# viiika/Diffusion-Conductor

Measured on AMD Instinct MI355X. Metric: motion frames/sec (DDIM-50, 60s clip, bs=32 per GPU), higher is better.
Workload: dtype f16; 1 GPU; configs[1]: DDIM-50 sampling loop, bs=32 clips/GPU x 1800 frames (60 s), linear attention, precision=fp16, conditioning + x_T resident in HBM (loop-only); clips_per_gpu=32, frames_per_clip=1800, ddim_steps=50, parallelism=clip-dp1, precise_tail_steps=1

## Files before the change

### diffusion-conductor_amd/csrc/dc_api.hip

```cpp
#include <hip/hip_runtime.h>

#include <algorithm>
#include <cmath>
#include <cstdarg>
#include <cstdio>
#include <cstdlib>
#include <cstring>
#include <map>
#include <string>
#include <tuple>
#include <vector>

#include "../../include/dc_ddim.h"
#include "dc_common.h"
#include "dc_form.h"
#include "dc_launch.h"
#include "dc_music.h"
#include "dc_pack.h"

namespace {

thread_local std::string g_err;

int fail(int code, const char* fmt, ...) {
// ... 33 lines not shown
    DcModel* d_model = nullptr;
    DcModel h_model{};
    int NT = 0;

    hipStream_t stream = nullptr;
    hipEvent_t ev_in = nullptr, ev_out = nullptr;

    int B = 0, T = 0, M = 0, G = 0;
    int Tx = 0;
    size_t cap_G = 0, cap_B = 0, cap_MP = 0, cap_steps = 0, cap_snap = 0, cap_kv = 0;
    size_t cap_rec_floats = 0;
    std::vector<int> len_dev;
    const int* len_dev_ptr = nullptr;
    int* d_length = nullptr;
    float* d_pp = nullptr;
    void *d_s_hi = nullptr, *d_s_lo = nullptr;
    void* d_E = nullptr;
    float* d_h = nullptr;
    float* d_recs = nullptr;
    void *d_a_sa = nullptr, *d_a_ca = nullptr;
    void* d_a_ca16 = nullptr;
    unsigned long long* d_gran = nullptr;
    unsigned l16_seq = 0;
    bool l16_own = false;
    void *d_kv_sa[2] = {nullptr, nullptr}, *d_kv_ca = nullptr;
    int KT = 0;
    float* d_x = nullptr;
    float* d_snaps = nullptr;
    float* d_recs_ca = nullptr;
    void *d_nh_hi = nullptr, *d_nh_lo = nullptr;
    unsigned long long* d_stamps = nullptr;
    float* d_film_rate = nullptr;
    int film_rate_parity = 0;
    int num_cu = 0;
    int *d_iter = nullptr, *d_t_clip = nullptr, *d_snap_cur = nullptr, *d_t_of_iter = nullptr, *d_snap_of_iter = nullptr;
    float *d_coef_cur = nullptr, *d_coef_of_iter = nullptr;
    bool cond_set = false;
    int64_t ws_bytes = 0;
    std::map<void*, size_t> alloc_bytes;
    int tables_S = 0;
    std::vector<int> tab_t, tab_snap;
    std::vector<float> tab_coef_iter;

    std::vector<std::pair<GraphKey, hipGraphExec_t>> graphs;
    int upd_flags = 0;
    const float** d_zslot = nullptr;
    float* d_zstep = nullptr;
    size_t cap_zstep = 0;
    unsigned long long noise_seed = 0, noise_first = 0;
    bool noise_seed_set = false;
    int* d_status = nullptr;
    float* d_x0_prev = nullptr;
    size_t cap_x0_prev = 0;
    const float *known_val = nullptr, *known_mask = nullptr, *known_noise = nullptr;
    struct KnownFor {
        int user_B = 0, Tx = 0;
        bool guided = false;
        int takes = 1;
        bool operator==(const KnownFor& o) const { return user_B == o.user_B && Tx == o.Tx && guided == o.guided && takes == o.takes; }
    } known_set_for;
    KnownFor known_for() const { return {user_B(), Tx, guided, takes}; }
    const float** d_kslot = nullptr;
    int smooth_window = 0, smooth_order = 0, smooth_table_window = 0;
    float* d_smooth_coef = nullptr;
    bool guided = false;
    float guide_w = 1.f;
    float* d_wslot = nullptr;
    float* d_raw = nullptr;
    size_t cap_raw = 0;
    float *d_xf2_proj = nullptr, *d_xf2_out = nullptr;
    size_t cap_xf2_proj = 0, cap_xf2_out = 0;
    int user_B() const { return guided ? B / 2 : B; }
    int takes = 1;
    float* d_pp_share = nullptr;
    size_t cap_pp_share = 0;
    const float* pp_last = nullptr;
    int last_film_groups = 0;

    DcModel h_model_split{};
    DcModel* d_model_split = nullptr;
    dc_music* music = nullptr;
    int me_format = -1;
    int clip_aligned = -1;
    bool precise_forward = false;
    int tail_split = -1;
    bool host_only = false;

    Prof prof;
    bool diag_film_done = false;
};

namespace {

template <class P>
int dev_alloc(dc_sampler* s, P*& p, size_t bytes) {
    if (p) {
        auto it = s->alloc_bytes.find((void*)p);
        if (it != s->alloc_bytes.end()) {
            s->ws_bytes -= (int64_t)it->second;
            s->alloc_bytes.erase(it);
        }
        void* old = (void*)p;
        p = nullptr;
        HIP_TRY(hipFree(old));
    }
    void* q = nullptr;
    HIP_TRY(hipMalloc(&q, bytes));
    p = (P*)q;
    s->alloc_bytes[q] = bytes;
    s->ws_bytes += (int64_t)bytes;
    return DC_OK;
}

void drop_graph(dc_sampler* s) {
    for (auto& g : s->graphs) hipGraphExecDestroy(g.second);
    s->graphs.clear();
}

template <class P>
int grow(dc_sampler* s, P*& p, size_t& cap, size_t need, size_t elem_bytes, bool in_graphs) {
    if (need <= cap) return DC_OK;
    if (in_graphs) drop_graph(s);
    cap = 0;
    if (int rc = dev_alloc(s, p, need * elem_bytes)) return rc;
    cap = need;
    return DC_OK;
}

const std::vector<float>* find(dc_sampler* s, const std::string& n) {
    auto it = s->params.find(n);
    return it == s->params.end() ? nullptr : &it->second;
}

struct ParamReq {
    std::string name;
    size_t numel;
};

std::vector<ParamReq> required_params(const dc_config& c) {
    std::vector<ParamReq> r;
    const size_t D = c.latent_dim, E = 4 * D, L = 512, F = c.ff_size, P = c.input_feats;
    r.push_back({"sequence_embedding", (size_t)c.num_frames * D});
    r.push_back({"linear.weight", L * 64});
    r.push_back({"linear.bias", L});
    r.push_back({"joint_embed.weight", D * P});
    r.push_back({"joint_embed.bias", D});
    r.push_back({"time_embed.0.weight", E * D});
    r.push_back({"time_embed.0.bias", E});
    r.push_back({"time_embed.2.weight", E * E});
    r.push_back({"time_embed.2.bias", E});
    auto styl = [&](const std::string& p) {
        r.push_back({p + ".emb_layers.1.weight", 2 * D * E});
        r.push_back({p + ".emb_layers.1.bias", 2 * D});
        r.push_back({p + ".norm.weight", D});
        r.push_back({p + ".norm.bias", D});
        r.push_back({p + ".out_layers.2.weight", D * D});
        r.push_back({p + ".out_layers.2.bias", D});
    };
    for (int i = 0; i < c.num_layers; ++i) {
        const std::string p = "temporal_decoder_blocks." + std::to_string(i);
        r.push_back({p + ".sa_block.norm.weight", D});
        r.push_back({p + ".sa_block.norm.bias", D});
        for (const char* n : {"query", "key", "value"}) {
            r.push_back({p + ".sa_block." + n + ".weight", D * D});
            r.push_back({p + ".sa_block." + n + ".bias", D});
        }
// ... 292 lines not shown
        add_image(I.top(&DcModel::img_out), P("out.weight"), P_, DC_D, true, ob.data(), ob.size());
        std::vector<float> ob16(32, 0.f);
        for (int k = 0; k < P_; ++k) ob16[k] = P("out.bias")[k];
        add_image16(I.top(&DcModel::out16), P("out.weight"), P_, DC_D, nullptr, 0, 0, true, ob16);
    }
    void conditioning_front(const LinearStats& lin) {
        const float* w = P("linear.weight");
        std::vector<float> wt((size_t)64 * 512);
        for (int k = 0; k < 512; ++k)
            for (int x = 0; x < 64; ++x) wt[(size_t)x * 512 + k] = w[(size_t)k * 64 + x];
        add_vec(I.top(&DcModel::lin_wt), wt);
        add_vec(I.top(&DcModel::lin_b), P("linear.bias"), 512);
        add_vec(I.top(&DcModel::lin_gram), lin.gram);
        add_natural(I.top(&DcModel::lin_pack), w, 512, 64, false);
    }
    void time_embedding() {
        add_vec(I.top(&DcModel::temb), std::vector<float>((size_t)c.max_timesteps * 512, 0.f));
        std::vector<float> fr(64);
        for (int k = 0; k < 64; ++k) fr[k] = (float)std::exp((double)((float)(-std::log(10000.0)) * (float)k / 64.f));
        std::vector<float> w0t((size_t)128 * 512), w2t((size_t)512 * 512);
        const float* w0 = P("time_embed.0.weight");
        const float* w2 = P("time_embed.2.weight");
        for (int o = 0; o < 512; ++o) {
            for (int x = 0; x < 128; ++x) w0t[(size_t)x * 512 + o] = w0[(size_t)o * 128 + x];
            for (int x = 0; x < 512; ++x) w2t[(size_t)x * 512 + o] = w2[(size_t)o * 512 + x];
        }
        I.freqs = I.arena.add(fr);
        I.w0t = I.arena.add(w0t);
        I.b0 = I.arena.add(P("time_embed.0.bias"), 512 * 4);
        I.w2t = I.arena.add(w2t);
        I.b2 = I.arena.add(P("time_embed.2.bias"), 512 * 4);
    }
};

void pack_model(const dc_config& c, const Formats& fmt, const DcParams& params, ModelImage& I) {
    const int L = c.num_layers;
    I.NT = 3 * L * DC_FILM_TILES_PER_BLOCK;
    I.model.num_layers = L;
    I.model.input_feats = c.input_feats;
    I.model.num_frames = c.num_frames;
    I.model.max_timesteps = c.max_timesteps;
    I.split = I.model;
    ModelPacker k{c, fmt, params, I};
    const LinearStats lin = centre_linear(k.P("linear.weight"), k.P("linear.bias"));
    for (int i = 0; i < L; ++i) k.decoder_layer(i, lin);
    k.film_stack();
    k.pose_projections();
    k.add_vec(I.top(&DcModel::seq_emb), k.P("sequence_embedding"), (size_t)c.num_frames * DC_D);
    k.conditioning_front(lin);
    k.time_embedding();
}

int upload_model(dc_sampler* s, ModelImage& I) {
    const std::vector<uint8_t>& host = I.arena.host;
    s->NT = I.NT;
    s->arena_bytes = host.size();
    if (s->host_only) {
        free(s->d_arena);
        s->d_arena = (uint8_t*)malloc(host.size());
        memcpy(s->d_arena, host.data(), host.size());
    } else {
        if (s->d_arena) hipFree(s->d_arena);
        HIP_TRY(hipMalloc((void**)&s->d_arena, host.size()));
        HIP_TRY(hipMemcpy(s->d_arena, host.data(), host.size(), hipMemcpyHostToDevice));
    }
    I.arena.resolve(s->d_arena);
    s->h_model = I.model;
    s->h_model_split = I.split;
    if (s->host_only) return DC_OK;
    if (!s->d_model) HIP_TRY(hipMalloc((void**)&s->d_model, sizeof(DcModel)));
    HIP_TRY(hipMemcpy(s->d_model, &s->h_model, sizeof(DcModel), hipMemcpyHostToDevice));
    if (!s->d_model_split) HIP_TRY(hipMalloc((void**)&s->d_model_split, sizeof(DcModel)));
    HIP_TRY(hipMemcpy(s->d_model_split, &s->h_model_split, sizeof(DcModel), hipMemcpyHostToDevice));
    const auto op = [&](size_t off) { return (const float*)(s->d_arena + off); };
    HIP_TRY(dc_launch_temb_table(s->stream, op(I.freqs), op(I.w0t), op(I.b0), op(I.w2t), op(I.b2), (float*)s->h_model.temb, s->cfg.max_timesteps));
    HIP_TRY(hipStreamSynchronize(s->stream));
    return DC_OK;
}

Settings settings_of(const dc_sampler* s) {
    Settings r;
    r.precision = s->cfg.precision, r.fmt = *s, r.no_eff = s->cfg.no_eff != 0, r.clip_aligned = s->clip_aligned, r.l16_own = s->l16_own;
    r.num_layers = s->cfg.num_layers, r.split_model = s->d_model_split != nullptr, r.film_w16 = s->h_model.film_w16 != nullptr;
    r.film_w16_tail = s->h_model.film_w16_tail != nullptr, r.l16_max_units = dc_layer16_max_units();
    return r;
}
int clip_stride(const dc_sampler* s, int B, int Tx) { return clip_stride(settings_of(s), Switches::read(), B, Tx, s->num_cu); }
int ensure_workspace(dc_sampler* s, int B, int Tx) {
    const int T = clip_stride(s, B, Tx);
    const int M = B * T, G = cdiv(M, 32), L = s->cfg.num_layers, P = s->cfg.input_feats;
    if ((size_t)G > s->cap_G) {
        drop_graph(s);
        const size_t g = (size_t)G;
        s->cap_G = 0;
        int rc;
        if ((rc = dev_alloc(s, s->d_pp, g * 32 * 64 * 8 * 4))) return rc;
        if ((rc = dev_alloc(s, s->d_s_hi, g * 32 * 64 * 16))) return rc;
        if ((rc = dev_alloc(s, s->d_s_lo, g * 32 * 64 * 16))) return rc;
        if ((rc = dev_alloc(s, s->d_E, g * s->NT * 64 * 32))) return rc;
        if ((rc = dev_alloc(s, s->d_h, g * 4 * 64 * 64))) return rc;
        HIP_TRY(hipMemset(s->d_h, 0, g * 4 * 64 * 64));
        s->cap_rec_floats = rec_capacity(g);
        if ((rc = dev_alloc(s, s->d_recs, s->cap_rec_floats * 4))) return rc;
        if ((rc = dev_alloc(s, s->d_nh_hi, g * 32 * 64 * 16))) return rc;
        if ((rc = dev_alloc(s, s->d_nh_lo, g * 32 * 64 * 16))) return rc;
        if (!s->cfg.no_eff && (rc = dev_alloc(s, s->d_recs_ca, (size_t)L * g * 2 * DC_REC_FLOATS * 4))) return rc;
        s->cap_G = g;
    }
    if (s->cfg.no_eff) {
        const int KT = (T + 31) / 32 + 1;
        const size_t need = (size_t)B * KT;
        if (need > s->cap_kv) {
            drop_graph(s);
            s->cap_kv = 0;
            int rc;
            for (int i = 0; i < 2; ++i)
                if ((rc = dev_alloc(s, s->d_kv_sa[i], need * 16384))) return rc;
            if ((rc = dev_alloc(s, s->d_kv_ca, (size_t)L * need * 16384))) return rc;
            s->cap_kv = need;
        }
        s->KT = KT;
    }
    if ((size_t)B > s->cap_B) {
        drop_graph(s);
        s->cap_B = 0;
        int rc;
        if ((rc = dev_alloc(s, s->d_length, (size_t)B * 4))) return rc;
        if ((rc = dev_alloc(s, s->d_t_clip, (size_t)B * 4))) return rc;
        if ((rc = dev_alloc(s, s->d_a_sa, (size_t)B * 16 * 1024))) return rc;
        if ((rc = dev_alloc(s, s->d_a_ca, (size_t)L * B * 16 * 1024))) return rc;
        if ((rc = dev_alloc(s, s->d_a_ca16, (size_t)L * B * 8 * 1024))) return rc;
        if ((rc = dev_alloc(s, s->d_gran, (size_t)B * 1024 * 8))) return rc;
        HIP_TRY(hipMemset(s->d_gran, 0, (size_t)B * 1024 * 8));
        s->cap_B = (size_t)B;
    }
    if ((size_t)M * P > s->cap_MP) {
        drop_graph(s);
        s->cap_MP = 0;
        int rc;
        if ((rc = dev_alloc(s, s->d_x, (size_t)M * P * 4))) return rc;
        s->cap_MP = (size_t)M * P;
    }
    if (!s->d_iter) {
        int rc;
        if ((rc = dev_alloc(s, s->d_stamps, (8 * 32 + 8 + 1024 + 1024 + 256 + 8 + 512) * 8))) return rc;
        if ((rc = dev_alloc(s, s->d_film_rate, 2 * 1024 * sizeof(float)))) return rc;
        HIP_TRY(hipMemset(s->d_film_rate, 0, 2 * 1024 * sizeof(float)));
        if ((rc = dev_alloc(s, s->d_status, 16))) return rc;
        HIP_TRY(hipMemset(s->d_status, 0, 16));
        if ((rc = dev_alloc(s, s->d_zslot, 32))) return rc;
        HIP_TRY(hipMemset(s->d_zslot, 0, 32));
        if ((rc = dev_alloc(s, s->d_kslot, 32))) return rc;
        HIP_TRY(hipMemset(s->d_kslot, 0, 32));
        if ((rc = dev_alloc(s, s->d_iter, 16))) return rc;
        if ((rc = dev_alloc(s, s->d_snap_cur, 16))) return rc;
        if ((rc = dev_alloc(s, s->d_coef_cur, DC_COEF * 4))) return rc;
    }
    if ((s->B != B || s->T != T) && s->d_gran)
        HIP_TRY(hipMemsetAsync(s->d_gran, 0, s->cap_B * 1024 * 8, s->stream));
    s->B = B;
    s->T = T;
    s->Tx = Tx;
    s->M = M;
    s->G = G;
    return DC_OK;
}

// ... 29 lines not shown
    } while (0)

struct Step : StepOpts {
    const float* x_src = nullptr;
    float* x_dst = nullptr;
};
struct StepDone {
    bool embedded_next = false;
    bool folded = false;
};

DcFilmArgs film_args(const dc_sampler* s, const float* pp, const int* t_clip) {
    DcFilmArgs f{};
    f.W = s->h_model.film_w, f.bias_ft = s->h_model.film_b, f.s_hi = s->d_s_hi, f.s_lo = s->d_s_lo, f.E = s->d_E, f.G = s->G, f.NT = s->NT;
    f.nround = s->NT / 16, f.pp = pp, f.temb = s->h_model.temb, f.t_clip = t_clip, f.T = s->T, f.B = s->B;
    f.W16 = s->h_model.film_w16, f.bias16 = s->h_model.film_b16, f.status = s->d_status;
    return f;
}

int enqueue_step(dc_sampler* s, hipStream_t st, const Step& c, const Switches& w, StepDone* done = nullptr) {
    static const bool want_stamps = getenv("DC_STAMPS") != nullptr;
    const int B = s->B, T = s->T, M = s->M, G = s->G, Tx = s->Tx;
    const StepForm f = step_form(Geometry{B, T, Tx, G, s->num_cu, s->cap_rec_floats}, settings_of(s), w, c, want_stamps);
    const bool folded = f.folded;
    const int fs = f.fs, ff = f.ff, graph_step = c.graph_step;
    const bool ss = f.ss, sf = s->split_film;
    const unsigned l16_tag = folded ? 16u * (unsigned)graph_step : (0x40000000u | (16u * (s->l16_seq++ & 0x3ffffffu)));
    if (!f.error.empty()) return fail(DC_ERR_INVALID, "%s", f.error.c_str());
    if (done) done->embedded_next = f.embed_next, done->folded = folded;
    const DcModel* dmod = (c.split && !s->split_small) ? s->d_model_split : s->d_model;
    const int* iter_base = folded ? s->d_iter : nullptr;
    const int* t_src = folded ? s->d_t_of_iter + graph_step : s->d_t_clip;
    const float* coef_src = folded ? s->d_coef_of_iter + DC_COEF * (size_t)graph_step : s->d_coef_cur;
    const int* snap_src = folded ? s->d_snap_of_iter + graph_step : s->d_snap_cur;
    if (c.loop_mode && !folded)
        LAUNCH(K_BEGIN, dc_launch_begin_step(st, s->d_iter, s->d_t_of_iter, s->d_coef_of_iter, s->d_snap_of_iter,
                                             s->d_t_clip, s->d_coef_cur, s->d_snap_cur, B));
    if (c.loop_mode && (s->upd_flags & DC_UPD_ZSTEP))
        LAUNCH(K_NOISE, dc_launch_step_noise(st, s->d_zstep, (size_t)s->user_B() * Tx * s->cfg.input_feats, 0, reinterpret_cast<const unsigned long long*>(s->d_zslot) + 1,
                                             iter_base, folded ? graph_step : 0,
                                             folded ? nullptr : s->d_snap_cur, 0));
    if (!f.fuse_silu)
        LAUNCH(K_SILU, dc_launch_silu_emb(st, ff, sf, s->d_pp, s->h_model.temb, s->d_t_clip, s->d_s_hi, s->d_s_lo, G, T, B));
    DcEmbedArgs ea{};
    if (f.fuse_embed) ea = DcEmbedArgs{dmod, c.x_src, s->d_h, s->d_recs, s->d_length, M, Tx, f.nwg, f.upc, ss ? 1 : 0, 0};
    if (f.fuse_extra) ea = DcEmbedArgs{s->d_model, c.x_src, s->d_h, s->d_recs, s->d_length, M, Tx, f.nwg, f.upc, 0, 1};
    DcFilmArgs fa = film_args(s, f.fuse_silu ? s->d_pp : nullptr, t_src);
    if (f.g1_tiles) fa.bias_ft = s->h_model.film_b_g1, fa.bias16 = s->h_model.film_b16_g1;
    if (f.film_tail) fa.W16 = s->h_model.film_w16_tail;
    s->last_film_groups = f.film_groups;
    fa.G = f.film_groups;
    if (f.guided && f.film_period < f.film_wrap) {
        if (!s->d_pp_share || (size_t)f.film_groups > s->cap_pp_share) return fail(DC_ERR_INVALID, "internal: no operand image for the shared takes of a guided step");
        fa.pp = s->d_pp_share;
    }
    s->pp_last = fa.pp;
    fa.clk = want_stamps ? s->d_stamps + 252 : nullptr;
    if (f.adapt) fa.rate_in = s->d_film_rate + 1024 * s->film_rate_parity, fa.rate_out = s->d_film_rate + 1024 * (s->film_rate_parity ^ 1);
    fa.iter_base = iter_base;
    fa.embed = (f.fuse_embed || f.fuse_extra) ? &ea : nullptr;
    const bool diag_skip_film = getenv("DC_DIAG_SKIP_FILM") && !f.fuse_embed && !f.fuse_extra && s->diag_film_done;
    s->diag_film_done = true;
    if (!diag_skip_film) LAUNCH(K_FILM, dc_launch_film_gemm(st, ff, sf, fa));
    s->film_rate_parity ^= 1;
    const int nl_run = f.nl_run;
    DcLayerArgs la{};
    la.dm = dmod, la.hbuf = s->d_h, la.E = s->d_E, la.NT = s->NT, la.recs = s->d_recs, la.length = s->d_length, la.xin = c.x_src, la.xout = c.x_dst;
    la.out_mode = (c.loop_mode && !f.guided) ? 1 : 0, la.coef_cur = coef_src, la.snap_cur = snap_src, la.snaps = s->d_snaps, la.iter_base = iter_base;
    la.M = M, la.T = T, la.G = G, la.B = B, la.Tx = Tx, la.e_groups = f.film_groups, la.e_period = f.film_period, la.e_wrap = f.film_wrap, la.e_magic = film_magic(f.film_period, f.film_wrap);
    if (f.guided) la.xout = s->d_raw;
    la.upd = DcUpdate{s->d_zslot, s->d_status, (c.loop_mode ? s->upd_flags : 0) | f.upd_flags, folded ? graph_step : -1, nullptr, s->d_kslot, s->d_x0_prev};
    DcLayerArgs la_stamps = la;
    la_stamps.upd.stamps = s->d_stamps;
    if (s->cfg.no_eff) {
        LAUNCH(K_EMBED, dc_launch_embed_front_full(st, fs, ss, dmod, c.x_src, s->d_h, s->d_kv_sa[0], M, T, B, s->KT));
        for (int l = 0; l < nl_run; ++l)
            LAUNCH(K_LAYER, dc_launch_layer_full(st, fs, ss, (want_stamps && l == 3) ? la_stamps : la, l, s->d_kv_sa[l & 1], s->d_kv_sa[(l + 1) & 1],
                                                 s->d_kv_ca, s->KT, (l == nl_run - 1) ? f.stop_stage : 0));
        if (f.guided)
            LAUNCH(K_GUIDE, dc_launch_guided_update(st, s->d_raw, c.x_dst, (size_t)s->user_B() * Tx * s->cfg.input_feats, coef_src, snap_src,
                                                    s->d_snaps, iter_base, s->d_wslot, la.upd));
        return DC_OK;
    }
    const DcLayerForm lf{fs, ss, f.wgr, f.narrow, f.g1_tiles, f.upc, f.rec_stride};
    if (f.fuse_embed || f.fuse_extra || c.embedded) {
    } else if (c.dbg.first >= 0)
        LAUNCH(K_EMBED, dc_launch_front_from_h(st, fs, ss, dmod, s->d_h, s->d_recs, s->d_length, M, T, G, B, c.dbg.first));
    else
        LAUNCH(K_EMBED, dc_launch_embed_front(st, lf, dmod, c.x_src, s->d_h, s->d_recs, s->d_length, M, T, G, B,
                                              want_stamps ? s->d_stamps + 256 : nullptr, Tx));
    for (int l = c.dbg.first >= 0 ? c.dbg.first : 0; l < nl_run; ++l) {
        if (f.layer16) {
            static const bool stamps16 = getenv("DC_L16_STAMPS") != nullptr;
            LAUNCH(K_LAYER, dc_launch_layer16(st, fs, (stamps16 && l == 3) ? la_stamps : la, l, s->d_a_ca16, f.upc16, f.rec_stride,
                                              l == 0 ? f.upc_narrow : f.upc16, l == 0 ? (size_t)2 * DC_REC_FLOATS : (size_t)DC_REC_FLOATS,
                                              f.l16_shared ? s->d_gran : nullptr, l16_tag, f.g1_tiles));
            continue;
        }
        if (!f.wgr) LAUNCH(K_COMBINE, dc_launch_attn_combine(st, fs, s->d_recs, s->d_a_sa, T, G, B, 1, 32));
        LAUNCH(K_LAYER, dc_launch_layer(st, lf, la, l, s->d_a_sa, s->d_a_ca, (l == nl_run - 1) ? f.stop_stage : 0,
                                        ((l == 3 || l == 4) && want_stamps) ? s->d_stamps : nullptr));
    }
    if (f.guided)
        LAUNCH(K_GUIDE, dc_launch_guided_update(st, s->d_raw, c.x_dst, (size_t)s->user_B() * Tx * s->cfg.input_feats, coef_src, snap_src,
                                                s->d_snaps, iter_base, s->d_wslot, la.upd));
    return DC_OK;
}

int sync_in(dc_sampler* s, hipStream_t user) {
    HIP_TRY(hipEventRecord(s->ev_in, user));
    HIP_TRY(hipStreamWaitEvent(s->stream, s->ev_in, 0));
    return DC_OK;
}
int sync_out(dc_sampler* s, hipStream_t user) {
    HIP_TRY(hipEventRecord(s->ev_out, s->stream));
    HIP_TRY(hipStreamWaitEvent(user, s->ev_out, 0));
    return DC_OK;
}

struct LoopCall {
    const float* d_noise = nullptr;
    float* d_out = nullptr;
    int n = 0;
    bool listed = false;
    const int32_t* h_timesteps = nullptr;
    const float* h_rows = nullptr;
    int flags = 0;
    const float* d_step_noise = nullptr;
    const int32_t* h_snap_iters = nullptr;
    int n_snap = 0;
    float* d_snaps = nullptr;
    bool profile = false;
    float* h_ms = nullptr;
    int32_t* h_count = nullptr;
    int n_kernels = 0;
    void* stream = nullptr;
};

int loop_validate(dc_sampler* s, const LoopCall& c, int& flags) {
    const int S = c.n;
    const float* h_coef = c.h_rows;
    const bool profile = c.profile;
    if (!s || !s->finalized) return fail(DC_ERR_INVALID, "sampler not finalized");
    if (!s->cond_set) return fail(DC_ERR_INVALID, "dc_sampler_set_conditioning must be called first");
    if (S < 1 || S > s->cfg.max_timesteps) return fail(DC_ERR_INVALID, "num_steps %d outside [1, max_timesteps=%d]", S, s->cfg.max_timesteps);
    if (!c.d_noise || !c.d_out || !h_coef) return fail(DC_ERR_INVALID, "null pointer argument");
    if ((flags & DC_UPD_EPS) && s->cfg.no_eff && !(flags & DC_UPD_NOISY) && !getenv("DC_ALLOW_EPSILON_NO_EFF_ETA0"))
        return fail(DC_ERR_UNSUPPORTED, "EPSILON model with full attention (no_eff) at eta = 0 is outside the 1e-3 parity bound (up to 1.3e-3); "
                                        "use linear attention, or eta > 0");
    if (s->known_mask && !(s->known_set_for == s->known_for())) s->known_val = s->known_mask = s->known_noise = nullptr;
    const bool known = s->known_mask != nullptr;
    if (known && S > 1 && !(h_coef[5] > 0.f))
        return fail(DC_ERR_INVALID, "known values are set: the loop needs the [S][8] table of dc_ddim_coefficients_known (slot 5 = sqrt(1 - abar_prev))");
    if (known && profile) return fail(DC_ERR_UNSUPPORTED, "dc_sampler_profile_loop does not run with known values set");
    if (known) flags |= DC_UPD_KNOWN;
    if (s->smooth_window > 0 && s->Tx < s->smooth_window)
        return fail(DC_ERR_INVALID, "smoothing window %d exceeds the %d frames of a clip", s->smooth_window, s->Tx);
    return DC_OK;
}

int loop_prepare(dc_sampler* s, const LoopCall& c, int& flags, size_t MP) {
    const int S = c.n, n_snap = c.n_snap;
    const int32_t *h_t = c.h_timesteps, *h_snap_iters = c.h_snap_iters;
    const float* h_coef = c.h_rows;
    int rc;
    if ((rc = ensure_steps(s, S))) return rc;
    if ((rc = grow(s, s->d_snaps, s->cap_snap, (size_t)n_snap * MP, 4, true))) return rc;
// ... 512 lines not shown
    int rc;
    if ((rc = grow(s, s->d_xf2_proj, s->cap_xf2_proj, irows * 64, 4, false))) return rc;
    if ((rc = grow(s, s->d_xf2_out, s->cap_xf2_out, irows * 64, 4, false))) return rc;
    hipStream_t user = (hipStream_t)stream;
    for (int j = 0; j < takes; ++j) {
        HIP_TRY(hipMemcpyAsync(s->d_xf2_proj + (size_t)j * rows * 64, d_xf_proj, rows * 64 * 4, hipMemcpyDeviceToDevice, user));
        HIP_TRY(hipMemcpyAsync(s->d_xf2_out + (size_t)j * rows * 64, d_xf_out, rows * 64 * 4, hipMemcpyDeviceToDevice, user));
    }
    if (guided) {
        DcNull64 np{}, no{};
        memcpy(np.v, h_null_proj, sizeof np.v);
        memcpy(no.v, h_null_out, sizeof no.v);
        HIP_TRY(dc_launch_fill_rows64(user, s->d_xf2_proj + crows * 64, crows, np));
        HIP_TRY(dc_launch_fill_rows64(user, s->d_xf2_out + crows * 64, crows, no));
    }
    std::vector<int32_t> len2;
    if (h_length)
        for (long long j = 0; j < Bi / B; ++j) len2.insert(len2.end(), h_length, h_length + B);
    if ((rc = set_conditioning(s, s->d_xf2_proj, s->d_xf2_out, h_length ? len2.data() : nullptr, (int)Bi, T, stream))) return rc;
    s->cond_set = false;
    if (guided) {
        if ((rc = grow(s, s->d_raw, s->cap_raw, irows * s->cfg.input_feats, 4, true))) return rc;
        if (!s->d_wslot && (rc = dev_alloc(s, s->d_wslot, 16))) return rc;
        s->guide_w = 1.f;
        const FilmShare sh = film_share(s->B, s->T, s->G, true, takes, !s->split_film, Switches{});
        if (sh.period < sh.wrap) {
            const size_t gbytes = (size_t)32 * 64 * 8 * 4;
            if ((rc = grow(s, s->d_pp_share, s->cap_pp_share, (size_t)sh.groups, gbytes, true))) return rc;
            char* dst = reinterpret_cast<char*>(s->d_pp_share);
            const char* src = reinterpret_cast<const char*>(s->d_pp);
            HIP_TRY(hipMemcpyAsync(dst, src, (size_t)sh.period * gbytes, hipMemcpyDeviceToDevice, user));
            HIP_TRY(hipMemcpyAsync(dst + (size_t)sh.period * gbytes, src + (size_t)sh.wrap * gbytes, gbytes, hipMemcpyDeviceToDevice, user));
        }
    }
    s->guided = guided;
    s->takes = takes;
    s->cond_set = true;
    return DC_OK;
}

int dc_sampler_set_conditioning_guided(dc_sampler* s, const float* d_xf_proj, const float* d_xf_out, const int32_t* h_length, int32_t B,
                                       int32_t T, const float* h_null_proj, const float* h_null_out, void* stream) {
    if (!s || !s->finalized) return fail(DC_ERR_INVALID, "sampler not finalized");
    if (!h_null_proj || !h_null_out) return fail(DC_ERR_INVALID, "guided conditioning: the null pair (h_null_proj[64], h_null_out[64]) is NULL");
    return set_conditioning_images(s, d_xf_proj, d_xf_out, h_length, B, T, 1, h_null_proj, h_null_out, stream);
}

int dc_sampler_set_conditioning_takes(dc_sampler* s, const float* d_xf_proj, const float* d_xf_out, const int32_t* h_length, int32_t B,
                                      int32_t T, int32_t takes, const float* h_null_proj, const float* h_null_out, void* stream) {
    if (!s || !s->finalized) return fail(DC_ERR_INVALID, "sampler not finalized");
    if (takes < 1) return fail(DC_ERR_INVALID, "takes=%d: a conditioning holds at least one take per music", takes);
    if ((h_null_proj != nullptr) != (h_null_out != nullptr))
        return fail(DC_ERR_INVALID, "takes: the null pair is both vectors (guided) or neither (unguided); one of h_null_proj, h_null_out is NULL");
    if (takes == 1 && !h_null_proj) return dc_sampler_set_conditioning(s, d_xf_proj, d_xf_out, h_length, B, T, stream);
    return set_conditioning_images(s, d_xf_proj, d_xf_out, h_length, B, T, takes, h_null_proj, h_null_out, stream);
}

int dc_sampler_set_guidance_scale(dc_sampler* s, float w) {
    if (!s) return fail(DC_ERR_INVALID, "null sampler");
    if (!std::isfinite(w)) return fail(DC_ERR_INVALID, "guidance scale must be finite");
    if (!s->guided) return fail(DC_ERR_INVALID, "dc_sampler_set_conditioning_guided must be called first: the scale belongs to a guided conditioning");
    s->guide_w = w;
    return DC_OK;
}

int dc_sampler_set_precise_tail(dc_sampler* s, int32_t steps) {
    if (!s) return fail(DC_ERR_INVALID, "null sampler");
    if (steps < -1) return fail(DC_ERR_INVALID, "precise tail: steps >= 0, or -1 for the precision's default");
    s->tail_split = steps;
    return DC_OK;
}

int32_t dc_precise_tail_default(int32_t precision) {
    return precise_tail_default(precision);
}

int dc_sampler_set_clip_aligned(dc_sampler* s, int32_t mode) {
    if (!s) return fail(DC_ERR_INVALID, "null sampler");
    if (mode < -1 || mode > 1) return fail(DC_ERR_INVALID, "clip-aligned units: 1 (always), 0 (flat units), -1 (the library's rule)");
    s->clip_aligned = mode;
    return DC_OK;
}

int dc_sampler_set_precise_forward(dc_sampler* s, int32_t on) {
    if (!s) return fail(DC_ERR_INVALID, "null sampler");
    s->precise_forward = on != 0;
    return DC_OK;
}

int dc_sampler_set_combine_exchange(dc_sampler* s, int32_t on) {
    if (!s) return fail(DC_ERR_INVALID, "null sampler");
    s->l16_own = on == 0;
    return DC_OK;
}

int dc_sampler_set_encoder_format(dc_sampler* s, int32_t format) {
    if (!s) return fail(DC_ERR_INVALID, "null sampler");
    if (format != DC_ME_SPLIT && format != DC_ME_FP16) return fail(DC_ERR_INVALID, "encoder format %d (DC_ME_SPLIT = 0, DC_ME_FP16 = 1)", format);
    s->me_format = format;
    if (s->music) dc_music_set_format(s->music, format);
    return DC_OK;
}

int dc_sampler_encode_music(dc_sampler* s, const float* d_mel, int32_t B, int32_t Tm, int32_t n_mels, float* d_xf_proj,
                            float* d_xf_out, void* stream) {
    if (!s || !s->finalized) return fail(DC_ERR_INVALID, "sampler not finalized");
    if (!s->music) return fail(DC_ERR_PARAM, "music encoder parameters (music_encoder.*, proj.*) were not supplied");
    if (!d_mel || !d_xf_proj || !d_xf_out || B < 1) return fail(DC_ERR_INVALID, "bad encode_music arguments");
    if (n_mels != 128) return fail(DC_ERR_UNSUPPORTED, "mel spectrograms must have 128 bins (conv4 takes 32 channels x 16 bins), got %d", n_mels);
    if (Tm < 4) return fail(DC_ERR_INVALID, "need at least 4 mel frames (reflection padding of the (Tm - 1) / 3 + 1 rows behind the stride-3 pool), got %d", Tm);
    HIP_TRY(hipSetDevice(s->cfg.device));
    hipStream_t user = (hipStream_t)stream, st = s->stream;
    int rc;
    if ((rc = sync_in(s, user))) return rc;
    std::string err;
    const hipError_t e = dc_music_encode(s->music, d_mel, B, Tm, d_xf_proj, d_xf_out, st, &err);
    if (e != hipSuccess) return fail(DC_ERR_HIP, "encode_music: %s %s", hipGetErrorString(e), err.c_str());
    return sync_out(s, user);
}

int dc_savgol_coefficients(int32_t window, int32_t order, float* h_coef) {
    if (window < 3 || !(window & 1) || window > 99 || order < 0 || order >= window || order > 10 || !h_coef)
        return fail(DC_ERR_INVALID, "savgol: need an odd window in [3,99] and 0 <= order < window (order <= 10)");
    const int w = window, n = order + 1, hw = w / 2;
    std::vector<double> A((size_t)w * n), G((size_t)n * n, 0.0), Ginv((size_t)n * n, 0.0);
    for (int i = 0; i < w; ++i) {
        const double u = (double)(i - hw) / hw;
        double pw = 1.0;
        for (int j = 0; j < n; ++j) {
            A[(size_t)i * n + j] = pw;
            pw *= u;
        }
    }
    for (int a = 0; a < n; ++a)
        for (int b = 0; b < n; ++b) {
            double acc = 0.0;
            for (int i = 0; i < w; ++i) acc += A[(size_t)i * n + a] * A[(size_t)i * n + b];
            G[(size_t)a * n + b] = acc;
        }
    std::vector<double> M((size_t)n * 2 * n, 0.0);
    for (int a = 0; a < n; ++a) {
        for (int b = 0; b < n; ++b) M[(size_t)a * 2 * n + b] = G[(size_t)a * n + b];
        M[(size_t)a * 2 * n + n + a] = 1.0;
    }
    for (int c = 0; c < n; ++c) {
        int piv = c;
        for (int r = c + 1; r < n; ++r)
            if (std::fabs(M[(size_t)r * 2 * n + c]) > std::fabs(M[(size_t)piv * 2 * n + c])) piv = r;
        if (std::fabs(M[(size_t)piv * 2 * n + c]) < 1e-300) return fail(DC_ERR_INVALID, "savgol: singular normal equations");
        if (piv != c)
            for (int k = 0; k < 2 * n; ++k) std::swap(M[(size_t)piv * 2 * n + k], M[(size_t)c * 2 * n + k]);
        const double d = M[(size_t)c * 2 * n + c];
        for (int k = 0; k < 2 * n; ++k) M[(size_t)c * 2 * n + k] /= d;
        for (int r = 0; r < n; ++r)
            if (r != c) {
                const double f = M[(size_t)r * 2 * n + c];
                if (f != 0.0)
                    for (int k = 0; k < 2 * n; ++k) M[(size_t)r * 2 * n + k] -= f * M[(size_t)c * 2 * n + k];
            }
    }
    for (int a = 0; a < n; ++a)
        for (int b = 0; b < n; ++b) Ginv[(size_t)a * n + b] = M[(size_t)a * 2 * n + n + b];
    for (int i = 0; i < w; ++i)
        for (int k = 0; k < w; ++k) {
            double acc = 0.0;
            for (int a = 0; a < n; ++a) {
// ... 243 lines not shown
```

### diffusion-conductor_amd/csrc/dc_form.h

```cpp
#pragma once
#include <algorithm>
#include <cstdio>
#include <cstdlib>
#include <optional>
#include <string>
#include <tuple>
#include <vector>

#include "dc_common.h"

constexpr int DCF_BF16 = 0, DCF_MIXED = 1, DCF_BF16X3 = 2, DCF_FP16 = 3;

struct Formats {
    int small_fmt = 0, film_fmt = 0;
    bool split_small = false, split_film = false;
    void set_precision(int precision) {
        split_small = precision == DCF_MIXED || precision == DCF_BF16X3;
        split_film = precision == DCF_BF16X3;
        small_fmt = precision == DCF_FP16 ? 1 : 0;
        film_fmt = (precision == DCF_FP16 || precision == DCF_MIXED) ? 1 : 0;
    }
};

#define DC_FORM_SWITCHES(X)                                                                                                            \
    X(no_wgrec, "DC_NO_WGREC") X(no_narrow, "DC_NO_NARROW") X(no_align, "DC_NO_ALIGN") X(align, "DC_ALIGN")                          \
    X(no_fuse_embed, "DC_NO_FUSE_EMBED") X(film_static, "DC_FILM_STATIC") X(begin_step, "DC_BEGIN_STEP") X(no_pad, "DC_NO_PAD")      \
    X(no_layer16, "DC_NO_LAYER16") X(l16_own_combine, "DC_L16_OWN_COMBINE") X(l16_test_drop_slice, "DC_L16_TEST_DROP_SLICE")         \
    X(tail_film_bf16, "DC_TAIL_FILM_BF16") X(flat_units, "DC_FLAT_UNITS") X(no_embed_next, "DC_NO_EMBED_NEXT")                  \
    X(guide_full_film, "DC_GUIDE_FULL_FILM") X(takes_full_film, "DC_TAKES_FULL_FILM")
struct Switches {
#define X(field, name) bool field = false;
    DC_FORM_SWITCHES(X)
#undef X
    static Switches read() {
        Switches w;
#define X(field, name) w.field = getenv(name) != nullptr;
        DC_FORM_SWITCHES(X)
#undef X
        return w;
    }
    unsigned long long bits() const {
        unsigned long long k = 0;
        int i = 0;
#define X(field, name) k |= (field ? 1ull : 0ull) << i++;
        DC_FORM_SWITCHES(X)
#undef X
        return k;
    }
};

inline size_t rec_capacity(size_t g) { return std::max(g * 2, 4 * ((g + 3) / 4) + 8) * DC_REC_FLOATS; }

struct Geometry {
    int B = 0, T = 0, Tx = 0, G = 0;
    int num_cu = 0;
    size_t cap_rec_floats = 0;
};

inline unsigned long long guided_key_bits(bool guided, bool shared_film) {
    return (guided ? 1ull << 27 : 0ull) | ((guided && shared_film) ? 1ull << 28 : 0ull);
}

struct Settings {
    int precision = DCF_FP16;
    Formats fmt;
    bool no_eff = false;
    int clip_aligned = -1;
    bool l16_own = false;
    int num_layers = 0;
    bool split_model = false;
    bool film_w16 = false, film_w16_tail = false;
    int l16_max_units = 0;
};

struct Hooks {
    int layers = -1, stage = 0;
    int first = -1;
    bool production() const { return layers < 0 && stage == 0 && first < 0; }
};

struct StepOpts {
    bool loop_mode = false;
    int graph_step = -1;
    bool split = false;
    bool g1_loop = false;
    bool next_plain = false;
    bool embedded = false;
    bool profile = false;
    bool known = false;
    int takes = 1;
    bool guided = false;
    Hooks dbg;
};

struct StepForm {
    std::string error;
    bool ss = false;
    bool film_tail = false;
    int fs = 0, ff = 0;
    bool fuse_silu = false;
    bool folded = false;
    bool adapt = false;
    bool wgr = false, narrow = false, aligned = false, layer16 = false, l16_shared = false;
    int upc = 0, upc16 = 0, upc_narrow = 0, nwg = 0;
    size_t rec_stride = 0;
    bool mixed_form = false, embed_next = false, fuse_embed = false, fuse_extra = false, g1_tiles = false;
    int upd_flags = 0;
    int nl_run = 0, stop_stage = 0;
    bool guided = false;
    bool shared_film = false;
    int film_groups = 0;
    int film_period = 0, film_wrap = 0;
};

struct FilmShare {
    int period = 0, wrap = 0, groups = 0;
};
inline FilmShare film_share(int B, int T, int G, bool guided, int takes, bool film_from_pp, const Switches& w) {
    const FilmShare full{G, G, G};
    const int Bc = guided ? B / 2 : B;
    if ((guided && B % 2) || takes < 1 || Bc % takes || !film_from_pp || (guided && w.guide_full_film)) return full;
    const long long mc = (long long)(Bc / takes) * T;
    if (mc % 32 != 0) return full;
    const long long gc = mc / 32, wrap = gc * takes;
    if ((guided ? 2 * wrap : wrap) != G) return full;
    const int period = (int)((takes > 1 && !w.takes_full_film && gc >= 2 && wrap * gc < (1ll << 32)) ? gc : wrap), groups = period + (guided ? 1 : 0);
    return groups < G ? FilmShare{period, (int)wrap, groups} : full;
}
inline unsigned film_magic(int period, int wrap) { return period < wrap ? (unsigned)((1ull << 32) / (unsigned)period) + 1u : 0u; }
inline int takes_key_period(const FilmShare& f) { return f.period < f.wrap ? f.period : 0; }

inline bool can_split_steps(const Settings& s, const Hooks& dbg) {
    return (s.precision == DCF_FP16 || s.precision == DCF_BF16) && dbg.production() && s.split_model;
}

inline StepForm step_form(const Geometry& g, const Settings& s, const Switches& w, const StepOpts& o, bool stamps) {
    StepForm f;
    const int B = g.B, T = g.T, G = g.G;
    const Hooks& dbg = o.dbg;
    if (o.guided && !(o.loop_mode && B % 2 == 0 && dbg.production())) {
        f.error = "internal: a guided evaluation is a loop step over an even number of internal clips";
        return f;
    }
    const bool guided = f.guided = o.guided;
    const bool quiet = dbg.production() && !stamps;
    const bool ss = f.ss = s.fmt.split_small || o.split, sf = s.fmt.split_film;
    f.film_tail = o.split && !s.fmt.split_small && s.film_w16_tail && !w.tail_film_bf16;
    const int fs = f.fs = s.fmt.small_fmt, ff = f.ff = f.film_tail ? 1 : s.fmt.film_fmt;
    const bool fuse_silu = f.fuse_silu = !sf && dbg.layers < 0;
    f.folded = o.loop_mode && o.graph_step >= 0 && fuse_silu && !s.no_eff && !w.begin_step && dbg.stage == 0;
    f.adapt = !w.film_static && g.num_cu <= 1024;
    if (o.takes < 1 || (guided ? B / 2 : B) % o.takes != 0) {
        f.error = "internal: the conditional clips are not a whole number of takes";
        return f;
    }
    const FilmShare share = film_share(B, T, G, guided, o.takes, fuse_silu, w);
    f.film_groups = share.groups, f.film_period = share.period, f.film_wrap = share.wrap;
    f.shared_film = f.film_groups < G;
    f.nl_run = (dbg.layers >= 0 && dbg.layers < s.num_layers) ? dbg.layers : s.num_layers;
    f.stop_stage = s.no_eff ? (dbg.stage ? dbg.stage : (f.nl_run < s.num_layers ? 3 : 0)) : dbg.stage;
    const bool wgr = f.wgr = T >= 256 && !w.no_wgrec && dbg.first < 0 && !s.no_eff && (!ss || (T % 32 == 0 && dbg.production() && !w.no_align));
    const bool can_align = wgr && T % 32 == 0 && !w.no_align;
    const int upc_wide = (T + 255) / 256, upc_narrow = f.upc_narrow = (T + 127) / 128;
    const bool aligned_env = can_align && w.align;
    const int nwg_narrow = can_align ? B * upc_narrow : (G + 3) / 4;
    const bool narrow = f.narrow = wgr && !ss && nwg_narrow <= g.num_cu && T <= 3840 && quiet && !w.no_narrow;
    const int nwg_flat = (G + 7) / 8, ncu = g.num_cu > 0 ? g.num_cu : 256;
    const bool same_rounds = ((long long)B * upc_wide + ncu - 1) / ncu == ((long long)nwg_flat + ncu - 1) / ncu;
    const bool aligned_wide = s.clip_aligned > 0 || aligned_env || (s.clip_aligned < 0 && same_rounds && !w.flat_units);
    const bool aligned = f.aligned = can_align && (narrow || ss || aligned_wide);
    const int upc16 = f.upc16 = (T + 63) / 64;
    const bool layer16 = f.layer16 = narrow && aligned && (long long)B * upc16 <= g.num_cu && upc16 <= s.l16_max_units && dbg.first < 0 && !w.no_layer16;
    const int upc = f.upc = aligned ? (narrow ? upc_narrow : upc_wide) : 0;
    const int nwg = f.nwg = aligned ? B * upc : (narrow ? (G + 3) / 4 : (G + 7) / 8);
    f.l16_shared = layer16 && !s.l16_own && !w.l16_own_combine;
    f.rec_stride = wgr ? (size_t)nwg * 2 * DC_REC_FLOATS : 0;
    const size_t rec_floats = wgr ? 2 * f.rec_stride : (size_t)G * 2 * DC_REC_FLOATS;
    if (rec_floats > g.cap_rec_floats) {
        char buf[160];
        snprintf(buf, sizeof buf, "unit records of this launch form (%zu floats) exceed the workspace (%zu)", rec_floats, g.cap_rec_floats);
        f.error = buf;
        return f;
    }
    const bool mixed_form = f.mixed_form = ss && !sf && ff == 1 && fs == 0;
    const bool wide_plain = wgr && !narrow && !ss && fuse_silu && ff == fs && quiet && !s.no_eff;
    f.embed_next = !w.no_embed_next && o.loop_mode && o.next_plain && wide_plain && !guided;
    if (o.embedded && !(o.loop_mode && wide_plain)) {
        f.error = "internal: a step whose front work was done by its predecessor changed its launch form";
        return f;
    }
    f.fuse_embed = !o.embedded && wgr && !narrow && (ss ? (aligned && mixed_form) : ff == fs) && fuse_silu && quiet && nwg <= g.num_cu &&
                   !o.profile && !w.no_fuse_embed && !f.shared_film;
    f.fuse_extra = narrow && aligned && !ss && ff == fs && fuse_silu && s.film_w16 && dbg.first < 0 && !o.profile && !w.no_fuse_embed &&
                   !f.shared_film;
    f.upd_flags = (w.l16_test_drop_slice ? DC_UPD_TEST_DROP_SLICE : 0) | (f.embed_next ? DC_UPD_EMBED_NEXT : 0) |
                  ((o.known && o.loop_mode) ? DC_UPD_KNOWN : 0);
#ifndef DC_NO_FILM_G1
    f.g1_tiles = o.g1_loop && !ss && wgr && !s.no_eff && quiet;
#endif
    return f;
}

inline int clip_stride(const Settings& s, const Switches& w, int B, int Tx, int num_cu) {
    if (Tx < 32 && !s.no_eff && !w.no_pad) return 32;
    if (s.no_eff || Tx < 256 || Tx % 32 == 0 || w.no_pad) return Tx;
    const int Tp = (Tx + 31) / 32 * 32;
    if (s.fmt.split_small) return Tp;
    const bool small_batch = (long long)B * ((Tp + 127) / 128) <= num_cu;
    const auto rounds = [&](int T) { return (((long long)B * T + 255) / 256 + num_cu - 1) / num_cu; };
    if (!small_batch && rounds(Tp) > rounds(Tx)) return Tx;
    return (small_batch || (Tp - Tx) * 50 <= Tx) ? Tp : Tx;
}

inline int steps_per_graph(int S) {
    if (S <= 64) return S;
    for (int k = 64; k >= 1; --k)
        if (S % k == 0) return k;
    return 1;
}

#ifndef DC_BF16_TAIL_DEFAULT
#define DC_BF16_TAIL_DEFAULT 6
#endif
#ifndef DC_BF16_SHORT_CLIP
#define DC_BF16_SHORT_CLIP 100
#endif
inline int precise_tail_default(int precision) { return precision == DCF_FP16 ? 1 : precision == DCF_BF16 ? DC_BF16_TAIL_DEFAULT : 0; }

struct LoopTail {
    int tail;
    bool tail_all;
};
inline LoopTail loop_tail(const Settings& s, int tail_split, std::optional<int> env_tail, int flags, int Tx, int S) {
    int tail = tail_split >= 0 ? tail_split : precise_tail_default(s.precision);
    bool tail_asked = tail_split >= 0;
    if (env_tail) tail = *env_tail, tail_asked = true;
    if (!tail_asked && (flags & DC_UPD_EPS)) tail = S;
    if (!tail_asked && s.precision == DCF_BF16 && Tx < DC_BF16_SHORT_CLIP) tail = S;
    if (!can_split_steps(s, Hooks{})) tail = 0;
    const bool tail_all = tail >= S;
    return {std::max(0, std::min(tail, std::min(S, steps_per_graph(S)))), tail_all};
}

using GraphKey = std::tuple<int, int, int, int, unsigned long long, int>;

struct LoopOpts {
    int S = 1;
    int flags = 0;
    bool guided = false;
    int takes = 1;
    bool profile = false;
    bool no_graph = false;
    int tail_split = -1;
    std::optional<int> env_tail;
};
struct LoopPart {
    int steps = 0;
    int split_n = 0;
    int launches = 1;
    GraphKey key{};
};
struct LoopPlan {
    bool g1_loop = false;
    bool eager = false;
    std::vector<LoopPart> parts;
};
inline LoopPlan loop_plan(const Geometry& g, const Settings& s, const Switches& w, const LoopOpts& o) {
    const LoopTail lt = loop_tail(s, o.tail_split, o.env_tail, o.flags, g.Tx, o.S);
    LoopPlan p;
    p.g1_loop = lt.tail > 0, p.eager = o.profile || o.no_graph;
    if (p.eager) {
        p.parts.push_back({o.S, lt.tail_all ? o.S : lt.tail, 1, GraphKey{}});
        return p;
    }
    const FilmShare share = film_share(g.B, g.T, g.G, o.guided, o.takes, !s.fmt.split_film, w);
    const unsigned long long bits = w.bits() | (unsigned long long)(o.flags & 0xff) << 16 | (s.l16_own ? 1ull : 0ull) << 24 |
                                    (unsigned long long)((s.clip_aligned + 1) & 3) << 25 | guided_key_bits(o.guided, share.groups < g.G) |
                                    (p.g1_loop ? 1ull : 0ull) << 39;
    const int K = steps_per_graph(o.S), replays = o.S / K;
    const auto part = [&](int split_n, int launches) {
        p.parts.push_back({K, split_n, launches, GraphKey{g.B, g.T, g.Tx, K, bits | (unsigned long long)split_n << 40, takes_key_period(share)}});
    };
    if (lt.tail && replays > 1) {
        part(lt.tail_all ? K : 0, replays - 1);
        part(lt.tail, 1);
    } else {
        part(replays == 1 ? lt.tail : (lt.tail_all ? K : 0), replays);
    }
    return p;
}
inline StepOpts loop_step(const LoopPlan& p, const LoopPart& part, const LoopOpts& o, int i) {
    StepOpts c;
    c.loop_mode = true, c.graph_step = p.eager ? -1 : i, c.split = i >= part.steps - part.split_n, c.g1_loop = p.g1_loop;
    c.next_plain = i + 1 < part.steps - part.split_n, c.profile = o.profile, c.known = (o.flags & DC_UPD_KNOWN) != 0;
    c.guided = o.guided, c.takes = o.takes;
    return c;
}
```

### diffusion-conductor_amd/csrc/dc_kernels.hip

```cpp
#include "dc_dev.h"


__global__ void k_begin_step(int* __restrict__ iter, const int* __restrict__ t_of_iter,
                             const float* __restrict__ coef_of_iter, const int* __restrict__ snap_of_iter,
                             int* __restrict__ t_clip, float* __restrict__ coef_cur, int* __restrict__ snap_cur, int B) {
    const int it = *iter;
    const int t = t_of_iter[it];
    for (int b = threadIdx.x; b < B; b += blockDim.x) t_clip[b] = t;
    if (threadIdx.x < DC_COEF) coef_cur[threadIdx.x] = coef_of_iter[it * DC_COEF + threadIdx.x];
    __syncthreads();
    if (threadIdx.x == 0) {
        snap_cur[0] = snap_of_iter ? snap_of_iter[it] : -1;
        snap_cur[1] = it;
        *iter = it + 1;
    }
}

__global__ void k_advance_iter(int* __restrict__ iter, int k) { *iter += k; }
__global__ void k_set_ptr(const float** slot, const float* p, unsigned long long seed, unsigned long long first) {
    slot[0] = p;
    reinterpret_cast<unsigned long long*>(slot)[1] = seed;
    reinterpret_cast<unsigned long long*>(slot)[2] = first;
}

// ... 1043 lines not shown
        const RowRange vr[2] = {valid_rows_clip(cx, ub0, B, M, T, length, active), valid_rows_clip(cx, ub0 + 1, B, M, T, length, active)};
        asm volatile("s_waitcnt vmcnt(0)" ::: "memory");
        __syncthreads();
        stamp(3);
        f32x16 K[4];
#pragma unroll
        for (int oc = 0; oc < 4; ++oc) {
            K[oc] = splat(bk[32 * oc + cx.c]);
            mmb_oc<4, 4, T16, SPLIT>(K[oc], lk, oc, nf, lane);
        }
        wg_put_maxes<NW>(K, cx, vr, mx, wave);
        __syncthreads();
        stamp(4);
        const int s0 = cx.b0 - ub0;
        RowRange vr_own = vr[0];
        if (s0) vr_own = vr[1];
#pragma unroll
        for (int oc = 0; oc < 4; ++oc) {
            f32x16 V = splat(bv[32 * oc + cx.c]);
            mmb_oc<4, 4, T16, SPLIT>(V, lv, oc, nf, lane);
            float ssum;
            f32x8 keep;
            partial_tile<T16, SPLIT>(K[oc], V, vr_own, wg_colmax<NW>(mx, oc, s0, cx.c), cx, ssum, keep);
            pst[(wave * 4 + oc) * 64 + lane] = keep;
            if (cx.hh == 0) ss[(wave * 4 + oc) * 32 + cx.c] = ssum;
            if (!SPLIT && active && cx.straddle) {
                partial_tile<T16, SPLIT>(K[oc], V, vr[1], wg_colmax<NW>(mx, oc, 1, cx.c), cx, ssum, keep);
                xp[oc * 64 + lane] = keep;
                if (cx.hh == 0) ss[(NW * 4 + oc) * 32 + cx.c] = ssum;
            }
            __builtin_amdgcn_sched_barrier(0);
        }
        stamp(5);
        __syncthreads();
        stamp(6);
        wg_write_record<NW>(recs, mx, pst, xp, ss, wave, lane, ub0, wm.nact, wm.Mu, wm.Tu, wg);
        stamp(7);
    }
}
template <class T16, bool SPLIT, bool WGR, bool FROMH = false, bool NARROW = false>
__global__ __launch_bounds__((NARROW || (SPLIT && !WGR)) ? 256 : 512, (SPLIT && !WGR) ? 1 : 2)
void k_embed_front(const DcModel* __restrict__ dm, const float* __restrict__ x, float* __restrict__ hbuf, float* __restrict__ recs,
                   const int* __restrict__ length, int M, int T, int G, int B, unsigned long long* __restrict__ clk, int l0, int Tx, int upc) {
    embed_front_body<T16, SPLIT, WGR, FROMH, NARROW>(dm, x, hbuf, recs, length, M, T, G, B, clk, l0, Tx, upc, -1);
}
template <class T16, class TS = T16, bool SP = false>
__global__ __launch_bounds__(512, 2) void k_film_embed(const v8<T16>* __restrict__ W, const float* __restrict__ bias16,
                                                       f16x16* __restrict__ E, int G, int NT, int round0, int nround,
                                                       const float* __restrict__ pp, const float* __restrict__ temb,
                                                       const int* __restrict__ t_clip, int T, int B,
                                                       unsigned long long* __restrict__ clk, const float* __restrict__ rate_in,
                                                       float* __restrict__ rate_out, const int* __restrict__ iter_base, const DcEmbedArgs ea,
                                                       int* __restrict__ status) {
    const unsigned long long t_begin = __builtin_amdgcn_s_memrealtime();
    if constexpr (!SP) {
        if (ea.extra) {
            const int nf = (int)gridDim.x - ea.ne;
            if ((int)blockIdx.x >= nf) {
                if (threadIdx.x >= 256) return;
                embed_front_body<TS, false, true, false, true>(ea.dm, ea.x, ea.hbuf, ea.recs, ea.length, ea.M, T, G, B, nullptr, 0, ea.Tx, ea.upc,
                                                               (int)blockIdx.x - nf);
                return;
            }
            film_gemm3_body<T16>(W, bias16, E, G, NT, round0, nround, pp, temb, t_clip, T, B, clk, rate_in, rate_out, iter_base, t_begin, status, nf);
            return;
        }
    }
    if ((int)blockIdx.x < ea.ne) {
        embed_front_body<TS, SP, true, false, false>(ea.dm, ea.x, ea.hbuf, ea.recs, ea.length, ea.M, T, G, B, nullptr, 0, ea.Tx, ea.upc,
                                                     (int)blockIdx.x);
        asm volatile("s_waitcnt vmcnt(0) lgkmcnt(0)" ::: "memory");
        __syncthreads();
    }
    film_gemm3_body<T16>(W, bias16, E, G, NT, round0, nround, pp, temb, t_clip, T, B, clk, rate_in, rate_out, iter_base, t_begin, status,
                         (int)gridDim.x);
}

#ifndef DC_SPLIT_STYL_PF
#define DC_SPLIT_STYL_PF 2
#endif
#ifndef DC_SPLIT_NW
#define DC_SPLIT_NW 8
#endif
template <class T16, bool SPLIT, bool DBG, bool STAMP, bool WGR, bool NARROW = false, bool G1 = false >
__global__ __launch_bounds__((NARROW || (SPLIT && DC_SPLIT_NW == 4)) ? 256 : 512, (SPLIT && DC_SPLIT_NW == 4) ? 1 : 2)
void k_layer(const DcModel* __restrict__ dm, int l, float* __restrict__ hbuf, const f16x16* __restrict__ E, int NT,
             const v8<T16>* __restrict__ a_sa , const v8<T16>* __restrict__ a_ca ,
             float* __restrict__ recs, const int* __restrict__ length, const float* __restrict__ xin,
             float* __restrict__ xout, int out_mode, const float* __restrict__ coef_cur, const int* __restrict__ snap_cur,
             float* __restrict__ snaps, int M, int T, int G, int B, int dbg,
             unsigned long long* __restrict__ stamps, size_t rec_stride, const int* __restrict__ iter_base,
             int Tx , int upc ,
             int e_groups , int e_period, int e_wrap, unsigned e_magic , const DcUpdate upd) {
    extern __shared__ __attribute__((aligned(16))) char lds[];
    static_assert(!NARROW || (WGR && !SPLIT && !DBG), "narrow workgroups: workgroup-record form, non-split formats, no test hooks");
    constexpr int NW = NARROW ? 4 : (SPLIT ? DC_SPLIT_NW : 8);
    constexpr int WM = SPLIT ? 2 : 1;
    constexpr int NFW = 32 * WM;
#define DC_STAMP(k)                                                                                        \
    do {                                                                                                   \
        if (STAMP && stamps && blockIdx.x == 3 && (threadIdx.x & 63) == 0 && l == 3)                       \
            stamps[(threadIdx.x >> 6) * 32 + (k)] = __builtin_amdgcn_s_memrealtime();                      \
    } while (0)
#define DC_WGSTAMP(e)                                                                                      \
    do {                                                                                                   \
        if (STAMP && stamps && threadIdx.x == 0 && (l == 3 || l == 4) && blockIdx.x < 256)                 \
            stamps[264 + ((l - 3) * 256 + blockIdx.x) * 2 + (e)] = __builtin_amdgcn_s_memrealtime();       \
    } while (0)
    constexpr int WSZ = (NFW + 1) * 1024;
    constexpr int OFF_AF = 2 * WSZ;
    constexpr int OFF_ER = OFF_AF + 16384;
    constexpr int OFF_SS = SPLIT ? OFF_AF + 16384 : OFF_ER + 8 * 8192;
    static_assert(!(SPLIT && WGR) || NW == 8, "split workgroup records: 8-wave workgroups");
    using W = v8<T16>;
    const unsigned long long t_first = STAMP ? __builtin_amdgcn_s_memrealtime() : 0ull;
#ifndef DC_NO_EARLY_ARGS
    {
        const unsigned grid_x = gridDim.x;
        asm("" : "+s"(T) : "s"(l), "s"(hbuf), "s"(E), "s"(recs), "s"(a_ca), "s"(NT), "s"(M), "s"(Tx), "s"(G), "s"(B), "s"(rec_stride), "s"(upc), "s"(grid_x));
    }
#endif
    const int nl = dm->num_layers;
    f32x16 h[4];
    {
        const int g0 = wg_map(WGR ? wg_index() : (int)blockIdx.x, threadIdx.x >> 6, NW, G, M, T, B, WGR ? upc : 0).g;
        load_h(h, hbuf, g0, threadIdx.x & 63);
    }
  {
    const int tid_ = threadIdx.x;
    const int wave = __builtin_amdgcn_readfirstlane(tid_ >> 6), lane = tid_ & 63;
    const int wg = WGR ? wg_index() : (int)blockIdx.x;
    const WgMap wm = wg_map(wg, wave, NW, G, M, T, B, WGR ? upc : 0);
    const int g = wm.g;
    const bool active = wm.active;
    const GroupCtx cx = make_ctx(g, lane, M, T);
    char* buf0 = lds;
    char* buf1 = lds + WSZ;
    const W* w0 = reinterpret_cast<const W*>(buf0);
    const W* w1 = reinterpret_cast<const W*>(buf1);
    const float* c0 = reinterpret_cast<const float*>(buf0 + NFW * 1024);
    const float* c1 = reinterpret_cast<const float*>(buf1 + NFW * 1024);
    const bool wg_lds = WGR || (!SPLIT && T >= NW * 32);
    const int ub0 = wm.ub0;
    char* ring = lds + OFF_ER + wave * 8192;
    auto stage_attn = [&](const W* a) {
        if constexpr (SPLIT) {
            stage_frags<NW>(a + (size_t)ub0 * 16 * 64, lds + OFF_AF, 16, wave, lane);
        } else {
            const int c1i = min(ub0 + 1, B - 1);
            stage_frags<NW>(a + (size_t)ub0 * 16 * 64, lds + OFF_AF, 8, wave, lane);
            stage_frags<NW>(a + (size_t)c1i * 16 * 64, lds + OFF_AF + 8192, 8, wave, lane);
        }
    };
    const W* af = reinterpret_cast<const W*>(lds + OFF_AF);
    const DcLayer& L = dm->layer[l];
    const bool last = l + 1 >= nl;
    const f16x8* Eg = reinterpret_cast<const f16x8*>(E) + ((size_t)film_tile_group(g, e_period, e_wrap, e_groups, e_magic) * NT + (size_t)l * 24) * 128;
    const W* acl = a_ca + (size_t)l * B * 16 * 64;
    const float* recs_in = recs + (size_t)(l & 1) * rec_stride;
    float* recs_out = recs + (size_t)((l + 1) & 1) * rec_stride;

    DC_STAMP(0);
    if (STAMP && stamps && blockIdx.x == 3 && (threadIdx.x & 63) == 0 && l == 3) stamps[(threadIdx.x >> 6) * 32 + 26] = __builtin_amdgcn_s_memtime();
    DC_WGSTAMP(0);
    if (STAMP && stamps && threadIdx.x == 0 && (l == 3 || l == 4) && blockIdx.x < 256) stamps[2576 + (l - 3) * 256 + blockIdx.x] = t_first;
    stage_frags<NW>(L.img_sa_q, buf0, NFW + 1, wave, lane);
    if constexpr (NARROW)
        wg_combine_attn_narrow<T16>(recs_in, reinterpret_cast<W*>(lds + OFF_AF), reinterpret_cast<float*>(buf1), ub0, wm.Mu, wm.Tu, tid_, wg);
    else if constexpr (WGR)
        wg_combine_attn<T16, SPLIT>(recs_in, reinterpret_cast<W*>(lds + OFF_AF), reinterpret_cast<float*>(buf1), ub0, B, wm.Mu, wm.Tu, tid_, wg,
                                    (STAMP && stamps && blockIdx.x == 3 && l == 3) ? stamps : nullptr);
    else if (wg_lds)
        stage_attn(a_sa);
    DC_STAMP(14);
    constexpr bool use_ring = !SPLIT;
#ifdef DC_PROLOGUE_WAIT_ALL
    if constexpr (use_ring) {
        ering_issue(Eg, 0, ring, lane);
        ering_issue(Eg, 1, ring + 4096, lane);
    }
    asm volatile("s_waitcnt vmcnt(0)" ::: "memory");
    DC_STAMP(15);
    stage_sync();
#else
    if constexpr (use_ring) {
        ering_issue(Eg, 0, ring, lane);
        ering_issue(Eg, 1, ring + 4096, lane);
#ifdef DC_DIAG_NO_ELOAD
        asm volatile("s_waitcnt vmcnt(0)" ::: "memory");
#else
        asm volatile("s_waitcnt vmcnt(8)" ::: "memory");
#endif
    } else {
        asm volatile("s_waitcnt vmcnt(0)" ::: "memory");
    }
    DC_STAMP(15);
    __builtin_amdgcn_sched_barrier(0);
    __syncthreads(); sprio<3>();
    __builtin_amdgcn_sched_barrier(0);
#endif
#ifdef DC_DIAG_HALF_SHIFT
    if constexpr (WGR && !SPLIT && !NARROW && !DBG) {
        if (wave >= NW / 2) { for (int i_ = 0; i_ < DC_DIAG_HALF_SHIFT; ++i_) __builtin_amdgcn_s_barrier(); }
        __builtin_amdgcn_sched_barrier(0);
    }
#endif
    DC_STAMP(1);

    stage_frags<NW>(L.img_sa_o, buf1, NFW + 1, wave, lane);
    EPre ep;
    constexpr bool split_pf = DC_SPLIT_STYL_PF && SPLIT && !DBG;
    EPf epf;
    if constexpr (use_ring) epre_load(ep, Eg, lane);
    ytile<SPLIT> y[4];
    float y_rstd, y_shift;
    const int skip_blocks = DBG ? (dbg >> 16) & 3 : 0;
    if (DBG && skip_blocks >= 1) {
    } else if (wg_lds)
        query_attend<T16, SPLIT>(y, y_rstd, y_shift, h, c0, w0, af + (SPLIT ? 0 : (size_t)(cx.b0 - ub0) * 8 * 64),
                                 af + (SPLIT ? 0 : (size_t)(cx.b1 - ub0) * 8 * 64), cx);
    else
        query_attend<T16, SPLIT>(y, y_rstd, y_shift, h, c0, w0, a_sa + (size_t)cx.b0 * 16 * 64,
                                 a_sa + (size_t)cx.b1 * 16 * 64, cx);
    DC_STAMP(2);
    if constexpr (split_pf && DC_SPLIT_STYL_PF == 2) {
        __builtin_amdgcn_sched_barrier(0);
        epf_fetch(epf, Eg, 0, 0, lane);
        epf_fetch(epf, Eg, 1, 1, lane);
        stage_sync_keep8();
    } else
        stage_sync();
    DC_STAMP(3);
    if constexpr (use_ring) epre_landed(ep);
    if constexpr (!use_ring) {
        stage_frags<NW>(L.img_ca_q, buf0, NFW + 1, wave, lane);
        if (wg_lds) stage_attn(acl);
        if (!(DBG && skip_blocks >= 1)) { if constexpr (split_pf) styl_accumulate_pf<T16, SPLIT, DC_SPLIT_STYL_PF == 2>(h, y, y_rstd, y_shift, Eg, epf, c1, w1, lane, cx.hh); else styl_accumulate<T16, SPLIT, G1>(h, y, y_rstd, y_shift, Eg, c1, w1, lane, cx.hh); }
    } else {
        auto next2 = [&]() {
            stage_frags<NW>(L.img_ca_q, buf0, NFW + 1, wave, lane);
            if (wg_lds) stage_attn(acl);
            ering_issue(Eg + 8 * 128, 0, ring, lane);
            ering_issue(Eg + 8 * 128, 1, ring + 4096, lane);
        };
        if (DBG && skip_blocks >= 1)
            next2();
        else
            styl_accumulate_ring<T16, SPLIT, G1>(h, y, y_rstd, y_shift, ep, ring, c1, w1, lane, cx.hh, next2);
    }
    if constexpr (DBG) if ((dbg & 0xff) == 1) { if (active) store_h(h, hbuf, g, lane); return; }
    DC_STAMP(4);
    stage_sync();
    DC_STAMP(5);
    stage_frags<NW>(L.img_ca_o, buf1, NFW + 1, wave, lane);
    if constexpr (use_ring) epre_load(ep, Eg + 8 * 128, lane);
    if (DBG && skip_blocks >= 2) {
    } else if (wg_lds)
        query_attend<T16, SPLIT>(y, y_rstd, y_shift, h, c0, w0, af + (SPLIT ? 0 : (size_t)(cx.b0 - ub0) * 8 * 64),
                                 af + (SPLIT ? 0 : (size_t)(cx.b1 - ub0) * 8 * 64), cx);
    else
        query_attend<T16, SPLIT>(y, y_rstd, y_shift, h, c0, w0, acl + (size_t)cx.b0 * 16 * 64,
                                 acl + (size_t)cx.b1 * 16 * 64, cx);
    DC_STAMP(6);
    if constexpr (split_pf && DC_SPLIT_STYL_PF == 2) {
        __builtin_amdgcn_sched_barrier(0);
        epf_fetch(epf, Eg + 8 * 128, 0, 0, lane);
        epf_fetch(epf, Eg + 8 * 128, 1, 1, lane);
        stage_sync_keep8();
    } else
        stage_sync();
    if constexpr (use_ring) epre_landed(ep);
    if constexpr (!use_ring) {
        stage_frags<NW>(L.img_ffn_w1, buf0, 16 * WM, wave, lane);
        stage_frags<NW>(L.img_ffn_w2, buf0 + 16 * WM * 1024, 16 * WM + 1, wave, lane);
        if (!(DBG && skip_blocks >= 2)) { if constexpr (split_pf) styl_accumulate_pf<T16, SPLIT, DC_SPLIT_STYL_PF == 2>(h, y, y_rstd, y_shift, Eg + 8 * 128, epf, c1, w1, lane, cx.hh); else styl_accumulate<T16, SPLIT, G1>(h, y, y_rstd, y_shift, Eg + 8 * 128, c1, w1, lane, cx.hh); }
    } else {
        auto next4 = [&]() {
            stage_frags<NW>(L.img_ffn_w1, buf0, 16 * WM, wave, lane);
            stage_frags<NW>(L.img_ffn_w2, buf0 + 16 * WM * 1024, 16 * WM + 1, wave, lane);
            ering_issue(Eg + 16 * 128, 0, ring, lane);
            ering_issue(Eg + 16 * 128, 1, ring + 4096, lane);
        };
        if (DBG && skip_blocks >= 2)
            next4();
        else
            styl_accumulate_ring<T16, SPLIT, G1>(h, y, y_rstd, y_shift, ep, ring, c1, w1, lane, cx.hh, next4);
    }
    if constexpr (DBG) if ((dbg & 0xff) == 2) { if (active) store_h(h, hbuf, g, lane); return; }
    DC_STAMP(7);
    stage_sync();
    DC_STAMP(8);
    stage_frags<NW>(L.img_ffn_o, buf1, NFW + 1, wave, lane);
    if constexpr (use_ring) epre_load(ep, Eg + 16 * 128, lane);
    {
        f32x16 u[2];
        {
            XFrag<T16, SPLIT> hf[4];
#pragma unroll
            for (int kt = 0; kt < 4; ++kt) make_frag<T16, SPLIT>(h[kt], hf[kt]);
#pragma unroll
            for (int t = 0; t < 2; ++t) u[t] = ld_ft(c0, t, cx.hh);
            gemm_wa<2, 4, T16, SPLIT>(u, w0, hf, lane);
        }
        sprio<2>();
        XFrag<T16, SPLIT> uf[2];
#pragma unroll
        for (int kt = 0; kt < 2; ++kt) {
#pragma unroll
            for (int r = 0; r < 8; ++r) {
                const f32x2 gg = gelu_erf_pair(u[kt][2 * r], u[kt][2 * r + 1]);
                u[kt][2 * r] = gg.x;
                u[kt][2 * r + 1] = gg.y;
            }
            make_frag<T16, SPLIT>(u[kt], uf[kt]);
        }
        RowStats st;
        sprio<1>();
#pragma unroll
        for (int t = 0; t < 4; ++t) {
            if (t == 2) sprio<0>();
            f32x16 yf = ld_ft(c0 + 64, t, cx.hh);
            mma_ot<4, 2, T16, SPLIT>(yf, w0 + 16 * WM * 64, t, uf, lane);
            st.add(yf);
            put_y<SPLIT>(y[t], yf);
        }
        st.finish(y_rstd, y_shift);
    }
    DC_STAMP(9);
    if constexpr (split_pf && DC_SPLIT_STYL_PF == 2) {
        __builtin_amdgcn_sched_barrier(0);
        epf_fetch(epf, Eg + 16 * 128, 0, 0, lane);
        epf_fetch(epf, Eg + 16 * 128, 1, 1, lane);
        stage_sync_keep8();
    } else
        stage_sync();
    if constexpr (use_ring) epre_landed(ep);
    {
        auto next_w = [&]() {
            if (!last)
                stage_frags<NW>(dm->layer[l + 1].img_sa_k, buf0, NFW + 1, wave, lane);
            else
                stage_frags<NW>(dm->img_out, buf0, 17, wave, lane);
        };
        if constexpr (!use_ring) {
            next_w();
            { if constexpr (split_pf) styl_accumulate_pf<T16, SPLIT, DC_SPLIT_STYL_PF == 2>(h, y, y_rstd, y_shift, Eg + 16 * 128, epf, c1, w1, lane, cx.hh); else styl_accumulate<T16, SPLIT, G1>(h, y, y_rstd, y_shift, Eg + 16 * 128, c1, w1, lane, cx.hh); }
        } else {
            styl_accumulate_ring<T16, SPLIT, G1>(h, y, y_rstd, y_shift, ep, ring, c1, w1, lane, cx.hh, next_w);
        }
    }
    if constexpr (DBG) if ((dbg & 0xff) == 3) { if (active) store_h(h, hbuf, g, lane); return; }
    DC_STAMP(10);
    stage_sync();
#ifdef DC_DIAG_HALF_SHIFT
    if constexpr (WGR && !SPLIT && !NARROW && !DBG) {
        if (wave < NW / 2) { for (int i_ = 0; i_ < DC_DIAG_HALF_SHIFT; ++i_) __builtin_amdgcn_s_barrier(); }
        __builtin_amdgcn_sched_barrier(0);
    }
#endif
    DC_STAMP(11);

    bool embed_next = false;
    if constexpr (WGR && !SPLIT && !NARROW && !DBG) embed_next = last && out_mode == 1 && (upd.flags & DC_UPD_EMBED_NEXT) != 0;
    if (last) {
    if (embed_next) {
        stage_frags<NW>(dm->layer[0].img_sa_k, buf1, NFW + 1, wave, lane);
        stage_frags<NW>(dm->img_je, lds + OFF_ER, 17, wave, lane);
    }
    f32x16 x0[1];
    const int P = dm->input_feats;
    const int e_xb = min(cx.tok, M - 1) / T, e_xn = cx.tok - e_xb * T;
    const bool e_live = cx.tok < M && e_xn < Tx;
    f32x4 sev[16];
    float xtv[16];
    {
        XFrag<T16, true> hf[4];
#pragma unroll
        for (int kt = 0; kt < 4; ++kt) make_frag<T16, true>(h[kt], hf[kt]);
        if (embed_next) {
            const size_t xrow = (size_t)e_xb * Tx + e_xn;
#pragma unroll
            for (int r = 0; r < 16; ++r) {
                const int f = tile_row(r, cx.hh);
                xtv[r] = (active && e_live && f < P) ? xin[xrow * P + f] : 0.f;
            }
        }
        x0[0] = ld_ft(reinterpret_cast<const float*>(buf0 + 16 * 1024), 0, cx.hh);
        gemm_wa<1, 4, T16, true>(x0, w0, hf, lane);
    }
    if (embed_next) {
        if constexpr (WGR && !SPLIT && !NARROW && !DBG) {
            __builtin_amdgcn_sched_barrier(0);
            asm volatile("s_waitcnt vmcnt(0)" ::: "memory");
            __syncthreads(); sprio<3>();
            __builtin_amdgcn_sched_barrier(0);
            stage_frags<NW>(dm->layer[0].img_sa_v, buf0, NFW + 1, wave, lane);
            const int xb = e_xb, xn = e_xn;
            const bool live = e_live;
            {
                const float* se = dm->seq_emb + (size_t)(e_live ? e_xn : 0) * DC_D;
#pragma unroll
                for (int t = 0; t < 4; ++t)
#pragma unroll
                    for (int q = 0; q < 4; ++q) sev[4 * t + q] = *reinterpret_cast<const f32x4*>(se + 32 * t + 8 * q + 4 * cx.hh);
            }
            f32x16 xv = splat(0.f);
            if (active && live) {
                const size_t xrow = (size_t)xb * Tx + xn;
                const int ib = iter_base ? *iter_base : 0;
                const float* cc = coef_cur + DC_COEF * ib;
                const int snap = snap_cur[ib];
                const bool noisy = (upd.flags & DC_UPD_NOISY) != 0;
                const float* zrow = nullptr;
                if (noisy) zrow = *upd.zslot + ((upd.flags & DC_UPD_ZSTEP) ? (size_t)0 : (size_t)(iter_base ? upd.step + ib : snap_cur[1]) * B * Tx * P);
                const KnownPtrs kn = known_ptrs(upd);
                bool bad = false;
#pragma unroll
                for (int r = 0; r < 16; ++r) {
                    const int f = tile_row(r, cx.hh);
                    if (f < P) {
                        const size_t o = xrow * P + f;
                        const float xnew = known_replace(multistep_update(x0[0][r], xtv[r], cc, upd, noisy, noisy ? zrow[o] : 0.f, bad, o), kn, o, cc);
                        xout[o] = xnew;
                        if (snap >= 0) snaps[(size_t)snap * B * Tx * P + o] = xnew;
                        xv[r] = xnew;
                    }
                }
                if (bad && upd.status) atomicOr(upd.status, DC_STATUS_NONFINITE);
            }
            if (active) {
                XFrag<T16, true> xf[1];
                make_frag<T16, true>(xv, xf[0]);
                const W* img = reinterpret_cast<const W*>(lds + OFF_ER);
                const float* je_b = reinterpret_cast<const float*>(img + 16 * 64);
#pragma unroll
                for (int t = 0; t < 4; ++t) h[t] = ld_ft(je_b, t, cx.hh);
                gemm_wa<4, 1, T16, true>(h, img, xf, lane);
#pragma unroll
                for (int t = 0; t < 4; ++t)
#pragma unroll
                    for (int q = 0; q < 4; ++q)
#pragma unroll
                        for (int i = 0; i < 4; ++i) h[t][4 * q + i] += sev[4 * t + q][i];
            }
            __builtin_amdgcn_sched_barrier(0);
        }
    } else {
    if (!active || cx.tok >= M) return;
    const int xb = cx.tok / T, xn = cx.tok - xb * T;
    if (xn >= Tx) return;
    const size_t xrow = (size_t)xb * Tx + xn;
    if (out_mode == 0) {
        bool bad = false;
#pragma unroll
        for (int r = 0; r < 16; ++r) {
            const int f = tile_row(r, cx.hh);
            if (f < P) {
                xout[xrow * P + f] = x0[0][r];
                bad = bad || !(fabsf(x0[0][r]) <= 3.0e38f);
            }
        }
        if (bad && upd.status) atomicOr(upd.status, DC_STATUS_NONFINITE);
    } else {
        const int ib = iter_base ? *iter_base : 0;
        coef_cur += DC_COEF * ib;
        const int snap = snap_cur[ib];
        const bool noisy = (upd.flags & DC_UPD_NOISY) != 0;
        const float* zrow = nullptr;
        if (noisy) zrow = *upd.zslot + ((upd.flags & DC_UPD_ZSTEP) ? (size_t)0 : (size_t)(iter_base ? upd.step + ib : snap_cur[1]) * B * Tx * P);
        const KnownPtrs kn = known_ptrs(upd);
        bool bad = false;
#pragma unroll
        for (int r = 0; r < 16; ++r) {
            const int f = tile_row(r, cx.hh);
            if (f < P) {
                const size_t o = xrow * P + f;
                const float xnew = known_replace(multistep_update(x0[0][r], xin[o], coef_cur, upd, noisy, noisy ? zrow[o] : 0.f, bad, o), kn, o, coef_cur);
                xout[o] = xnew;
                if (snap >= 0) snaps[(size_t)snap * B * Tx * P + o] = xnew;
            }
        }
        if (bad && upd.status) atomicOr(upd.status, DC_STATUS_NONFINITE);
    }
    return;
    }
    }
    {
        const DcLayer& Ln = dm->layer[last ? 0 : l + 1];
        char* const bufK = last ? buf1 : buf0;
        char* const bufV = last ? buf0 : buf1;
        const W* const wK = reinterpret_cast<const W*>(bufK);
        const W* const wV = reinterpret_cast<const W*>(bufV);
        const float* const cK = reinterpret_cast<const float*>(bufK + NFW * 1024);
        const float* const cV = reinterpret_cast<const float*>(bufV + NFW * 1024);
        if (!last) stage_frags<NW>(Ln.img_sa_v, bufV, NFW + 1, wave, lane);
        __builtin_amdgcn_sched_barrier(0);
#ifdef DC_DIAG_NO_HSTORE
        const bool st_h = false;
#else
        const bool st_h = active;
#endif
#ifdef DC_NO_STORE_STAGGER
        constexpr bool stagger = false;
#else
        constexpr bool stagger = WGR && !SPLIT && !NARROW && !DBG;
#endif
        const bool late_store = stagger && wave >= NW / 2;
        if (st_h && !late_store) store_h(h, hbuf, g, lane);
        __builtin_amdgcn_sched_barrier(0);
        XFrag<T16, SPLIT> nf[4];
        ln_frags<T16, SPLIT>(nf, h);
        DC_STAMP(19);
        if constexpr (WGR) {
            float* mx = reinterpret_cast<float*>(lds + OFF_AF);
            f32x8* pst = reinterpret_cast<f32x8*>(SPLIT ? bufK : lds + OFF_ER);
            f32x8* xp = reinterpret_cast<f32x8*>(lds + OFF_AF + 8192);
            float* ss = reinterpret_cast<float*>(lds + OFF_SS);
            float* scw = reinterpret_cast<float*>(SPLIT ? lds + OFF_AF + 8192 : bufK) + wave * 2 * 4 * 32;
            const RowRange vr0 = valid_rows_clip(cx, ub0, B, M, T, length, active);
            const RowRange vr1 = valid_rows_clip(cx, ub0 + 1, B, M, T, length, active);
            const int s0 = cx.b0 - ub0;
            const RowRange vr_own = s0 ? vr1 : vr0;
            const bool strad = !SPLIT && active && cx.straddle;
            XFrag<T16, SPLIT> efA[4], efB[SPLIT ? 1 : 4];
            float ssA[4], ssB[4], mA[4], mB[4];
            auto keys_of = [&](const f32x16& K, const RowRange& rr, XFrag<T16, SPLIT>& ef, float& ssum, float& mcol) {
                float m = -INFINITY;
                const bool full = __builtin_amdgcn_readfirstlane(rr.span) == 32u;
                if (full) {
                    m = max16(K);
                } else {
#pragma unroll
                    for (int r = 0; r < 16; ++r) m = row_ok(rr, r) ? fmaxf(m, K[r]) : m;
                }
                m = xhalf_max(m);
                mcol = m;
                const float mz = m == -INFINITY ? 0.f : m;
                f32x16 Ee;
                float sacc = 0.f;
                if (full) {
                    sacc = exp_rows(Ee, K, mz);
                } else {
#pragma unroll
                    for (int r = 0; r < 16; ++r) {
                        Ee[r] = row_ok(rr, r) ? exp2f_fast(K[r] - mz) : 0.f;
                        sacc += Ee[r];
                    }
                }
                ssum = xhalf_sum(sacc);
                make_frag<T16, SPLIT>(Ee, ef);
            };
            f32x16 Kp[4] = {splat(cK[cx.c]), splat(cK[32 + cx.c]), splat(cK[64 + cx.c]), splat(cK[96 + cx.c])};
            mmb_oc_quad<4, 4, T16, SPLIT>(Kp[0], Kp[1], Kp[2], Kp[3], wK, nf, lane);
            sprio<2, 2>();
#pragma unroll
            for (int q = 0; q < 4; ++q) {
                const int oc = q;
                if (q == 1) sprio<1, 2>();
                if (q == 3) sprio<0, 2>();
                keys_of(Kp[q], vr_own, efA[oc], ssA[oc], mA[oc]);
                mB[oc] = -INFINITY;
                if constexpr (!SPLIT)
                    if (strad) keys_of(Kp[q], vr1, efB[oc], ssB[oc], mB[oc]);
                if (cx.hh == 0) {
                    mx[((oc * 2 + s0) * 32 + cx.c) * NW + wave] = mA[oc];
                    mx[((oc * 2 + (s0 ^ 1)) * 32 + cx.c) * NW + wave] = s0 ? -INFINITY : mB[oc];
                }
            }
            __builtin_amdgcn_sched_barrier(0);
            DC_STAMP(20);
            if (st_h && late_store) {
                __builtin_amdgcn_sched_barrier(0);
                store_h(h, hbuf, g, lane);
                __builtin_amdgcn_sched_barrier(0);
            }
            if (st_h)
                asm volatile("s_waitcnt vmcnt(16)" ::: "memory");
            else
                asm volatile("s_waitcnt vmcnt(0)" ::: "memory");
            DC_STAMP(21);
            __syncthreads(); sprio<3>();
            __builtin_amdgcn_sched_barrier(0);
            DC_STAMP(12);
#pragma unroll
            for (int oc = 0; oc < 4; ++oc) {
                const float fa = mA[oc] == -INFINITY ? 0.f : exp2f_fast(mA[oc] - wg_colmax<NW>(mx, oc, s0, cx.c));
                ssA[oc] *= fa;
                if (cx.hh == 0) scw[(0 * 4 + oc) * 32 + cx.c] = fa;
                if (!SPLIT && strad) {
                    const float fb = mB[oc] == -INFINITY ? 0.f : exp2f_fast(mB[oc] - wg_colmax<NW>(mx, oc, 1, cx.c));
                    ssB[oc] *= fb;
                    if (cx.hh == 0) scw[(1 * 4 + oc) * 32 + cx.c] = fb;
                }
            }
            asm volatile("s_waitcnt lgkmcnt(0)" ::: "memory");
            const int rowq = 16 * (cx.c >> 4) + 4 * cx.hh;
            auto block_of = [&](const XFrag<T16, SPLIT>& ef, const f32x16& V, const RowRange& rr, const float* sc) {
                f32x16 Vm;
                if (__builtin_amdgcn_readfirstlane(rr.span) == 32u) {
                    Vm = V;
                } else {
#pragma unroll
                    for (int r = 0; r < 16; ++r) Vm[r] = row_ok(rr, r) ? V[r] : 0.f;
                }
                XFrag<T16, SPLIT> vf;
                make_frag<T16, SPLIT>(Vm, vf);
                f32x16 P = splat(0.f);
#pragma unroll
                for (int s2 = 0; s2 < 2; ++s2) {
                    P = mfma(ef.hi[s2], vf.hi[s2], P);
                    if constexpr (SPLIT) {
                        P = mfma(ef.lo[s2], vf.hi[s2], P);
                        P = mfma(ef.hi[s2], vf.lo[s2], P);
                    }
                }
                f32x8 keep = keep_head_block(P, cx.c);
                const f32x4 f0 = *reinterpret_cast<const f32x4*>(sc + rowq), f1 = *reinterpret_cast<const f32x4*>(sc + rowq + 8);
#pragma unroll
                for (int i = 0; i < 4; ++i) {
                    keep[i] *= f0[i];
                    keep[4 + i] *= f1[i];
                }
                return keep;
            };
            f32x16 Vp[4] = {splat(cV[cx.c]), splat(cV[32 + cx.c]), splat(cV[64 + cx.c]), splat(cV[96 + cx.c])};
            mmb_oc_quad<4, 4, T16, SPLIT>(Vp[0], Vp[1], Vp[2], Vp[3], wV, nf, lane);
            sprio<2, 2>();
#pragma unroll
            for (int q = 0; q < 4; ++q) {
                const int oc = q;
                if (q == 1) sprio<1, 2>();
                if (q == 3) sprio<0, 2>();
                pst[(wave * 4 + oc) * 64 + lane] = block_of(efA[oc], Vp[q], vr_own, scw + (0 * 4 + oc) * 32);
                if (cx.hh == 0) ss[(wave * 4 + oc) * 32 + cx.c] = ssA[oc];
                if constexpr (!SPLIT)
                    if (strad) {
                        xp[oc * 64 + lane] = block_of(efB[oc], Vp[q], vr1, scw + (1 * 4 + oc) * 32);
                        if (cx.hh == 0) ss[(NW * 4 + oc) * 32 + cx.c] = ssB[oc];
                    }
            }
            __builtin_amdgcn_sched_barrier(0);
            DC_STAMP(16);
            __syncthreads(); sprio<3>();
            DC_STAMP(17);
            wg_write_record<NW>(recs_out, mx, pst, xp, ss, wave, lane, ub0, wm.nact, wm.Mu, wm.Tu, wg);
        } else {
            f32x16 K[4];
#pragma unroll
            for (int oc = 0; oc < 4; ++oc) {
                K[oc] = splat(cK[32 * oc + cx.c]);
                mmb_oc<4, 4, T16, SPLIT>(K[oc], wK, oc, nf, lane);
            }
            __builtin_amdgcn_sched_barrier(0);
            if (st_h)
                asm volatile("s_waitcnt vmcnt(16)" ::: "memory");
            else
                asm volatile("s_waitcnt vmcnt(0)" ::: "memory");
            __syncthreads(); sprio<3>();
            __builtin_amdgcn_sched_barrier(0);
            DC_STAMP(12);
            float* rec = recs + (size_t)cx.g * 2 * DC_REC_FLOATS;
            const RowRange valid0 = valid_rows(cx, 0, M, T, length);
            const RowRange valid1 = valid_rows(cx, cx.straddle ? 1 : 0, M, T, length);
#pragma unroll
            for (int oc = 0; oc < 4; ++oc) {
                f32x16 V = splat(cV[32 * oc + cx.c]);
                mmb_oc<4, 4, T16, SPLIT>(V, wV, oc, nf, lane);
                if (active) {
                    emit_partial<T16, SPLIT>(K[oc], V, oc, valid0, rec, cx);
                    if (cx.straddle) emit_partial<T16, SPLIT>(K[oc], V, oc, valid1, rec + DC_REC_FLOATS, cx);
                }
                __builtin_amdgcn_sched_barrier(0);
            }
        }
        DC_STAMP(13);
        if (STAMP && stamps && blockIdx.x == 3 && (threadIdx.x & 63) == 0 && l == 3) stamps[(threadIdx.x >> 6) * 32 + 27] = __builtin_amdgcn_s_memtime();
        DC_WGSTAMP(1);
        return;
    }
  }
}

#ifndef DC_FULL_SUM_ADDS
#define DC_FULL_SUM_ADDS 2
#endif
#ifdef DC_DIAG_FULL_MOVES
__device__ unsigned long long g_full_moves[2];
hipError_t dc_full_moves_read(unsigned long long* out, bool reset) {
    hipError_t e = hipMemcpyFromSymbol(out, HIP_SYMBOL(g_full_moves), 16);
    if (e == hipSuccess && reset) {
        const unsigned long long z[2] = {0, 0};
        e = hipMemcpyToSymbol(HIP_SYMBOL(g_full_moves), z, 16);
    }
    return e;
}
#else
hipError_t dc_full_moves_read(unsigned long long* out, bool) {
    out[0] = out[1] = 0;
    return hipErrorNotSupported;
}
#endif
#define DC_FULL_ZOFF (32768 + 8 * 8192)
#define DC_FULL_LDS (DC_FULL_ZOFF + 8192)
struct ClipCtx {
    int b, g_lo, nkt, g, c, hh, tok, n;
    bool active, lane_ok;
};
DEV ClipCtx make_clip_ctx(int blk, int WPC, int wave, int lane, int T, int M) {
    ClipCtx x;
    x.b = blk / WPC;
    const int j = blk % WPC;
    x.g_lo = (x.b * T) / 32;
    const int g_hi = ((x.b + 1) * T - 1) / 32;
    x.nkt = g_hi - x.g_lo + 1;
    x.g = x.g_lo + j * 8 + wave;
    x.active = x.g <= g_hi;
    if (!x.active) x.g = g_hi;
    x.c = lane & 31;
    x.hh = lane >> 5;
    x.tok = 32 * x.g + x.c;
    x.n = x.tok - x.b * T;
    x.lane_ok = x.active && x.n >= 0 && x.n < T && x.tok < M;
    return x;
}
DEV void store_h_lanes(const f32x16 (&h)[4], float* __restrict__ hbuf, int g, int lane, bool ok) {
    if (ok) store_h(h, hbuf, g, lane);
}

template <class T16, bool SPLIT = false>
DEV void front_full(const XFrag<T16, SPLIT> (&nf)[4], const v8<T16>* __restrict__ wk, const v8<T16>* __restrict__ wv,
                    v8<T16>* __restrict__ tile, int lane, int c, int hh) {
    constexpr int HL = SPLIT ? 2 : 1;
    const float* bk = reinterpret_cast<const float*>(wk + 32 * 64 * HL);
    const float* bv = reinterpret_cast<const float*>(wv + 32 * 64 * HL);
#pragma unroll
    for (int t = 0; t < 4; ++t) {
        f32x16 K;
#pragma unroll
        for (int q = 0; q < 4; ++q) {
            const f32x4 v = *reinterpret_cast<const f32x4*>(bk + 32 * t + 8 * q + 4 * hh);
#pragma unroll
// ... 775 lines not shown
    const DcEmbedArgs* ea = a.embed;
    if (ea && ea->x && ea->extra) {
        if (ea->split_bf16 || ea->upc <= 0) return hipErrorInvalidValue;
        const int nf = film_extra_workgroups(nunit, nblk, ea->ne, ncu);
        if (nf <= 0) return hipErrorInvalidValue;
        static unsigned long long optin4 = 0;
        if (hipError_t e = lds_optin((const void*)k_film_embed<T16>, (int)shm, optin4)) return e;
        k_film_embed<T16><<<dim3(nf + ea->ne), dim3(512), shm, st>>>(W16, a.bias16, E, a.G, a.NT, a.round0, a.nround, a.pp, a.temb, a.t_clip, a.T,
                                                                     a.B, a.clk, a.rate_in, a.rate_out, a.iter_base, *ea, a.status);
        return hipGetLastError();
    }
    if (ea && ea->x && nwg >= ea->ne) {
        if (ea->split_bf16) {
            if (!std::is_same<T16, _Float16>::value || ea->upc <= 0) return hipErrorInvalidValue;
            const size_t shm2 = 8192 + 65 * 1024 + 9 * 4 * 32 * 4 + 65 * 1024;
            static unsigned long long optin3 = 0;
            if (hipError_t e = lds_optin((const void*)k_film_embed<T16, __bf16, true>, (int)shm2, optin3)) return e;
            k_film_embed<T16, __bf16, true><<<dim3(nwg), dim3(512), shm2, st>>>(W16, a.bias16, E, a.G, a.NT, a.round0, a.nround, a.pp, a.temb,
                                                                                a.t_clip, a.T, a.B, a.clk, a.rate_in, a.rate_out, a.iter_base, *ea,
                                                                                a.status);
            return hipGetLastError();
        }
        static unsigned long long optin2 = 0;
        if (hipError_t e = lds_optin((const void*)k_film_embed<T16>, (int)shm, optin2)) return e;
        k_film_embed<T16><<<dim3(nwg), dim3(512), shm, st>>>(W16, a.bias16, E, a.G, a.NT, a.round0, a.nround, a.pp, a.temb, a.t_clip, a.T, a.B,
                                                             a.clk, a.rate_in, a.rate_out, a.iter_base, *ea, a.status);
        return hipGetLastError();
    }
    if (ea && ea->x) return hipErrorInvalidValue;
    k_film_gemm3<T16><<<dim3(nwg), dim3(512), shm, st>>>(W16, a.bias16, E, a.G, a.NT, a.round0, a.nround, a.pp, a.temb, a.t_clip, a.T, a.B,
                                                         a.clk, a.rate_in, a.rate_out, a.iter_base, a.status);
    return hipGetLastError();
}
hipError_t dc_launch_film_gemm(hipStream_t st, int fmt, bool split, const DcFilmArgs& a) {
    if (!split && a.pp && a.W16) return fmt == 1 ? launch_film3_t<_Float16>(st, a) : launch_film3_t<__bf16>(st, a);
    if (a.embed && a.embed->x) return hipErrorInvalidValue;
    if (a.round0 != 0) return hipSuccess;
    DISPATCH(fmt, split, (launch_film_t<T16, SP>(st, a)));
    return LAUNCH_CHECK();
}

template <class T16, bool SP>
static hipError_t launch_front_from_h_t(hipStream_t st, const DcModel* dm, float* hbuf, float* recs, const int* length,
                                        int M, int T, int G, int B, int l0) {
    constexpr int NW = SP ? 4 : 8;
    k_embed_front<T16, SP, false, true><<<dim3((G + NW - 1) / NW), dim3(NW * 64), 0, st>>>(dm, nullptr, hbuf, recs, length, M, T, G, B, nullptr, l0, T, 0);
    return hipGetLastError();
}
hipError_t dc_launch_front_from_h(hipStream_t st, int fmt, bool split, const DcModel* dm, float* hbuf, float* recs, const int* length,
                                  int M, int T, int G, int B, int l0) {
    hipError_t e = hipSuccess;
    DISPATCH(fmt, split, (e = launch_front_from_h_t<T16, SP>(st, dm, hbuf, recs, length, M, T, G, B, l0)));
    return e;
}

template <class T16, bool SP, bool WGR, bool NARROW = false>
static hipError_t launch_embed_t(hipStream_t st, const DcModel* dm, const float* x, float* hbuf, float* recs, const int* length,
                                 int M, int T, int G, int B, unsigned long long* clk, int Tx, int upc) {
    constexpr int NW = (NARROW || (SP && !WGR)) ? 4 : 8;
    const size_t shm = !WGR ? 0 : SP ? 8192 + 65 * 1024 + 9 * 4 * 32 * 4 + 65 * 1024 : 8192 + 65536 + 8192 + 9 * 4 * 32 * 4 + 33 * 1024;
    if (WGR) {
        static unsigned long long optin_done = 0;
        if (hipError_t e = lds_optin((const void*)k_embed_front<T16, SP, WGR, false, NARROW>, (int)shm, optin_done)) return e;
    }
    k_embed_front<T16, SP, WGR, false, NARROW><<<dim3((WGR && upc) ? B * upc : (G + NW - 1) / NW), dim3(NW * 64), shm, st>>>(dm, x, hbuf, recs, length, M, T, G, B,
                                                                                                                         clk, 0, Tx, WGR ? upc : 0);
    return hipGetLastError();
}
#define EMBED_FORMS(X) X(false, false, false) X(true, false, false) X(false, true, false) X(false, true, true) X(true, true, false)
hipError_t dc_launch_embed_front(hipStream_t st, const DcLayerForm& f, const DcModel* dm, const float* x, float* hbuf, float* recs,
                                 const int* length, int M, int T, int G, int B, unsigned long long* clk, int Tx) {
    if (f.wgr && f.split && f.upc <= 0) return hipErrorInvalidValue;
#define X(SP, WGR, NARROW)                                                                                      \
    if (f.split == SP && f.wgr == WGR && f.narrow == NARROW)                                                    \
        return (f.fmt == 1 ? launch_embed_t<_Float16, SP, WGR, NARROW> : launch_embed_t<__bf16, SP, WGR, NARROW>)( \
            st, dm, x, hbuf, recs, length, M, T, G, B, clk, Tx, f.upc);
    EMBED_FORMS(X)
#undef X
    return hipErrorInvalidValue;
}

template <class T16, bool SP, bool DBG, bool STAMP, bool WGR, bool NARROW = false, bool G1 = false>
static hipError_t launch_layer_t(hipStream_t st, const DcLayerArgs& a, int l, const void* a_sa, const void* a_ca, int dbg,
                                 unsigned long long* stamps, size_t rec_stride, int upc) {
    constexpr int NW = NARROW ? 4 : (SP ? DC_SPLIT_NW : 8);
    const size_t shm = SP ? 2 * 65 * 1024 + (WGR ? 16384 + 6144 : 0) : 2 * 33 * 1024 + 16384 + 8 * 8192 + 6144;
    static unsigned long long optin_done = 0;
    if (hipError_t e = lds_optin((const void*)k_layer<T16, SP, DBG, STAMP, WGR, NARROW, G1>, (int)shm, optin_done)) return e;
    k_layer<T16, SP, DBG, STAMP, WGR, NARROW, G1><<<dim3((WGR && upc) ? a.B * upc : (a.G + NW - 1) / NW), dim3(NW * 64), shm, st>>>(
        a.dm, l, a.hbuf, (const f16x16*)a.E, a.NT, (const v8<T16>*)a_sa, (const v8<T16>*)a_ca, a.recs, a.length, a.xin, a.xout, a.out_mode,
        a.coef_cur, a.snap_cur, a.snaps, a.M, a.T, a.G, a.B, dbg, stamps, rec_stride, a.iter_base, a.Tx, WGR ? upc : 0, a.e_groups, a.e_period, a.e_wrap, a.e_magic, a.upd);
    return hipGetLastError();
}

#define LAYER_FORMS(X)                                                                                          \
    X(false, false, false, false, false, false) X(false, true, false, false, false, false) X(false, false, true, false, false, false) \
    X(true, false, false, false, false, false) X(true, true, false, false, false, false) X(true, false, true, false, false, false)    \
    X(false, false, false, true, false, false) X(false, true, false, true, false, false) X(false, false, true, true, false, false)    \
    X(false, false, false, true, false, true) X(false, false, false, true, true, false) X(false, false, false, true, true, true)      \
    X(true, false, false, true, false, false) X(true, false, true, true, false, false)
hipError_t dc_launch_layer(hipStream_t st, const DcLayerForm& f, const DcLayerArgs& a, int l, const void* a_sa, const void* a_ca, int dbg,
                           unsigned long long* stamps) {
    if (f.wgr && f.split && f.upc <= 0) return hipErrorInvalidValue;
    if (!a.tiles_ok()) return hipErrorInvalidValue;
    const bool stop = dbg != 0, stamp = stamps != nullptr && !stop;
#define X(SP, DBG, STAMP, WGR, NARROW, G1)                                                                      \
    if (f.split == SP && stop == DBG && stamp == STAMP && f.wgr == WGR && f.narrow == NARROW && f.g1 == G1)     \
        return (f.fmt == 1 ? launch_layer_t<_Float16, SP, DBG, STAMP, WGR, NARROW, G1> : launch_layer_t<__bf16, SP, DBG, STAMP, WGR, NARROW, G1>)( \
            st, a, l, a_sa, a_ca, dbg, stamps, f.rec_stride, f.upc);
    LAYER_FORMS(X)
#undef X
    return hipErrorInvalidValue;
}

template <class T16, bool SP>
static hipError_t launch_full_t(hipStream_t st, const DcLayerArgs& a, int l, const void* kv_cur, void* kv_next, const void* kv_ca, int KT,
                                int stop_after) {
    const int WPC = (KT + 7) / 8;
    static unsigned long long optin_done = 0;
    if (hipError_t e = lds_optin((const void*)k_layer_full<T16, SP>, DC_FULL_LDS, optin_done)) return e;
    k_layer_full<T16, SP><<<dim3(a.B * WPC), dim3(512), DC_FULL_LDS, st>>>(
        a.dm, l, a.hbuf, (const f16x16*)a.E, a.NT, (const v8<T16>*)kv_cur, (v8<T16>*)kv_next, (const v8<T16>*)kv_ca, a.length, a.xin, a.xout,
        a.out_mode, a.coef_cur, a.snap_cur, a.snaps, a.M, a.T, a.B, KT, WPC, stop_after, a.e_groups, a.e_period, a.e_wrap, a.e_magic, a.upd);
    return hipGetLastError();
}
hipError_t dc_launch_embed_front_full(hipStream_t st, int fmt, bool split, const DcModel* dm, const float* x, float* hbuf, void* kv_next,
                                      int M, int T, int B, int KT) {
    if (fmt != 1) return hipErrorInvalidValue;
    const int WPC = (KT + 7) / 8;
    if (split)
        k_embed_front_full<_Float16, true><<<dim3(B * WPC), dim3(512), 0, st>>>(dm, x, hbuf, (f16x8*)kv_next, M, T, KT, WPC);
    else
        k_embed_front_full<_Float16, false><<<dim3(B * WPC), dim3(512), 0, st>>>(dm, x, hbuf, (f16x8*)kv_next, M, T, KT, WPC);
    return hipGetLastError();
}
hipError_t dc_launch_layer_full(hipStream_t st, int fmt, bool split, const DcLayerArgs& a, int l, const void* kv_cur, void* kv_next,
                                const void* kv_ca, int KT, int stop_after) {
    if (fmt != 1 || !a.tiles_ok()) return hipErrorInvalidValue;
    return (split ? launch_full_t<_Float16, true> : launch_full_t<_Float16, false>)(st, a, l, kv_cur, kv_next, kv_ca, KT, stop_after);
}
hipError_t dc_launch_ca_kv(hipStream_t st, int fmt, const DcModel* dm, const void* nh_hi, const void* nh_lo, void* kv_ca,
                           int M, int T, int G, int B, int KT, int L) {
    const dim3 grid((G + 3) / 4, L);
    if (fmt != 1) return hipErrorInvalidValue;
    k_cond_ca_kv<_Float16><<<grid, dim3(256), 0, st>>>(dm, (const bf16x8*)nh_hi, (const bf16x8*)nh_lo, (f16x8*)kv_ca, M, T, G, B, KT);
    return hipGetLastError();
}

__global__ __launch_bounds__(256) void k_savgol(const float* __restrict__ x, float* __restrict__ y, const float* __restrict__ coef,
                                                int B, int T, int P, int win) {
    const long long idx = (long long)blockIdx.x * 256 + threadIdx.x;
    if (idx >= (long long)B * T * P) return;
    const int p = (int)(idx % P);
    const int t = (int)((idx / P) % T);
    const int b = (int)(idx / ((long long)P * T));
    const int h = win >> 1;
    int row, t0;
    if (t < h) {
        row = t;
        t0 = 0;
    } else if (t >= T - h) {
        row = win - (T - t);
        t0 = T - win;
    } else {
        row = h;
        t0 = t - h;
    }
    const float* c = coef + row * win;
    const float* src = x + ((size_t)b * T + t0) * P + p;
    float acc = 0.f;
    for (int k = 0; k < win; ++k) acc = fmaf(c[k], src[(size_t)k * P], acc);
    y[idx] = acc;
}
hipError_t dc_launch_savgol(hipStream_t st, const float* x, float* y, const float* coef, int B, int T, int P, int win) {
    const long long n = (long long)B * T * P;
    k_savgol<<<dim3((unsigned)((n + 255) / 256)), dim3(256), 0, st>>>(x, y, coef, B, T, P, win);
    return hipGetLastError();
}
```

### diffusion-conductor_amd/csrc/dc_launch.h

```cpp
#pragma once
#include <hip/hip_runtime.h>
#include "dc_common.h"

hipError_t dc_launch_begin_step(hipStream_t st, int* iter, const int* t_of_iter, const float* coef_of_iter,
                                const int* snap_of_iter, int* t_clip, float* coef_cur, int* snap_cur, int B);
hipError_t dc_launch_temb_table(hipStream_t st, const float* freqs, const float* w0t, const float* b0,
                                const float* w2t, const float* b2, float* temb, int nt);
hipError_t dc_launch_cond_embed(hipStream_t st, int mode, const float* xf, const float* wt, const float* b, float* out_f32,
                                void* out_hi, void* out_lo, int M, int G, int T ,
                                int Tx );
hipError_t dc_launch_ca_partials(hipStream_t st, const DcModel* dm, const void* nh_hi, const void* nh_lo,
                                 float* recs, int M, int T, int G, int L, int Tx );
hipError_t dc_launch_cond_pp64(hipStream_t st, const float* xf , const void* wpack, const float* b, float* out_f32, int M, int G, int T, int Tx);
hipError_t dc_launch_ca_partials64(hipStream_t st, const DcModel* dm, const float* xf , const float* gram, float* rstd, float* recs,
                                   int M, int T, int G, int L, int Tx);
hipError_t dc_launch_attn_combine(hipStream_t st, int fmt, const float* recs, void* afrag, int T, int NU, int B, int nset,
                                  int gran);
hipError_t dc_launch_silu_emb(hipStream_t st, int fmt, bool split, const float* pp, const float* temb, const int* t_clip,
                              void* s_hi, void* s_lo, int G, int T, int B,
                              const int* iter_base = nullptr );
struct DcFilmArgs {
    const void* W;
    const float* bias_ft;
    const void *s_hi, *s_lo;
    void* E;
    int G, NT, round0, nround;
    const float *pp, *temb;
    const int* t_clip;
    int T, B;
    unsigned long long* clk;
    const float* rate_in;
    float* rate_out;
    const int* iter_base;
    const void* W16;
    const float* bias16;
    const DcEmbedArgs* embed;
    int* status;
};
hipError_t dc_launch_film_gemm(hipStream_t st, int fmt, bool split, const DcFilmArgs& a);
struct DcLayerForm {
    int fmt;
    bool split;
    bool wgr;
    bool narrow;
    bool g1;
    int upc;
    size_t rec_stride;
};
hipError_t dc_launch_embed_front(hipStream_t st, const DcLayerForm& f, const DcModel* dm, const float* x, float* hbuf, float* recs,
                                 const int* length, int M, int T, int G, int B,
                                 unsigned long long* clk ,
                                 int Tx );
hipError_t dc_launch_front_from_h(hipStream_t st, int fmt, bool split, const DcModel* dm, float* hbuf, float* recs, const int* length,
                                  int M, int T, int G, int B, int l0);
struct DcLayerArgs {
    const DcModel* dm;
    float* hbuf;
    const void* E;
    int NT;
    float* recs;
    const int* length;
    const float* xin;
    float* xout;
    int out_mode;
    const float* coef_cur;
    const int* snap_cur;
    float* snaps;
    const int* iter_base;
    int M, T, G, B;
    int Tx;
    int e_groups;
    int e_period, e_wrap;
    unsigned e_magic;
    DcUpdate upd;
    bool tiles_ok() const { return e_period >= 1 && e_wrap >= e_period && e_groups >= 1 && e_period <= e_groups && (e_magic != 0) == (e_period < e_wrap); }
};
hipError_t dc_launch_layer(hipStream_t st, const DcLayerForm& f, const DcLayerArgs& a, int l, const void* a_sa, const void* a_ca,
                           int dbg ,
                           unsigned long long* stamps );
hipError_t dc_launch_layer16(hipStream_t st, int fmt, const DcLayerArgs& a, int l, const void* a_ca16, int upc, size_t rec_stride, int nu_in,
                             size_t stride_in,
                             unsigned long long* gran ,
                             unsigned tag_base ,
                             bool g1 );
hipError_t dc_launch_cond_af16(hipStream_t st, int fmt, const void* a_ca, void* a_ca16, int n_matrices);
int dc_layer16_max_units(void);
hipError_t dc_launch_advance_iter(hipStream_t st, int* iter, int k);
hipError_t dc_launch_set_ptr(hipStream_t st, const float** slot , const float* p, unsigned long long seed,
                             unsigned long long first);
hipError_t dc_launch_set_known(hipStream_t st, const float** slot, const float* val, const float* mask, const float* noise);
hipError_t dc_launch_known_blend(hipStream_t st, float* x, const float* val, const float* mask, const float* noise, float ca, float cb, size_t n);
hipError_t dc_launch_fill_rows64(hipStream_t st, float* dst, size_t rows, const DcNull64& v);
hipError_t dc_launch_set_scale(hipStream_t st, float* slot, float w);
hipError_t dc_launch_guided_update(hipStream_t st, const float* raw, float* x, size_t n, const float* coef_cur, const int* snap_cur, float* snaps,
                                   const int* iter_base, const float* wslot, const DcUpdate& upd);
hipError_t dc_launch_step_noise(hipStream_t st, float* z, size_t n, unsigned long long seed, const unsigned long long* seed_slot, const int* iter_base,
                                int step, const int* snap_cur, unsigned long long first);
hipError_t dc_launch_scan_f16(hipStream_t st, const void* e, size_t bytes, int* status);

hipError_t dc_launch_ca_kv(hipStream_t st, int fmt, const DcModel* dm, const void* nh_hi, const void* nh_lo, void* kv_ca,
                           int M, int T, int G, int B, int KT, int L);
hipError_t dc_launch_embed_front_full(hipStream_t st, int fmt, bool split, const DcModel* dm, const float* x, float* hbuf, void* kv_next,
                                      int M, int T, int B, int KT);
hipError_t dc_launch_layer_full(hipStream_t st, int fmt, bool split, const DcLayerArgs& a, int l, const void* kv_cur, void* kv_next,
                                const void* kv_ca, int KT, int stop_after);

hipError_t dc_full_moves_read(unsigned long long* out , bool reset);

hipError_t dc_launch_savgol(hipStream_t st, const float* x, float* y, const float* coef, int B, int T, int P, int win);
```

### diffusion-conductor_amd/native.py

```python
from __future__ import annotations

import ctypes as C
import os
import subprocess

import numpy as np

_HERE = os.path.dirname(os.path.abspath(__file__))
LIB_PATH = os.path.join(_HERE, "libdc_ddim.so")
CSRC = os.path.join(_HERE, "csrc")

DC_PREC = {"bf16": 0, "mixed": 1, "bf16x3": 2, "fp16": 3}

EXPORTS = [
    "dc_last_error", "dc_version", "dc_linear_beta_schedule", "dc_ddim_coefficients", "dc_pack_weight",
    "dc_sampler_create", "dc_sampler_destroy", "dc_sampler_set_param", "dc_sampler_finalize_params",
    "dc_sampler_set_conditioning", "dc_sampler_encode_music", "dc_sampler_set_encoder_format", "dc_sampler_set_precise_tail", "dc_precise_tail_default", "dc_sampler_set_precise_forward", "dc_sampler_set_combine_exchange", "dc_sampler_set_clip_aligned", "dc_sampler_denoise", "dc_sampler_ddim_loop", "dc_sampler_profile_loop",
    "dc_kernel_name", "dc_kernel_count", "dc_sampler_workspace_bytes", "dc_sampler_clip_stride", "dc_sampler_debug_denoise",
    "dc_sampler_debug_read", "dc_sampler_debug_layer", "dc_savgol_coefficients", "dc_savgol_filter",
    "dc_ddim_coefficients_ex", "dc_sampler_ddim_loop_ex", "dc_sampler_status", "dc_sampler_set_smoothing",
    "dc_sampler_set_step_noise_seed", "dc_sampler_set_step_noise_seed_at", "dc_step_noise_fill",
    "dc_motion_encoder_create", "dc_motion_encoder_destroy", "dc_motion_encoder_set_param", "dc_motion_encoder_finalize",
    "dc_motion_encoder_encode",
    "dc_ddim_coefficients_known", "dc_sampler_set_known",
    "dc_sampler_set_conditioning_guided", "dc_sampler_set_guidance_scale",
    "dc_m2snet_create", "dc_m2snet_destroy", "dc_m2snet_set_param", "dc_m2snet_finalize", "dc_m2snet_encode_music", "dc_m2snet_fuse",
    "dc_m2snet_score",
    "dc_solver_table", "dc_sampler_solver_loop", "dc_sampler_solver_profile_loop",
    "dc_sampler_set_conditioning_takes",
    "dc_q_sample_coefficients", "dc_q_sample", "dc_motion_loss_terms", "dc_latent_l1",
    "dc_m2sgan_create", "dc_m2sgan_destroy", "dc_m2sgan_set_param", "dc_m2sgan_finalize", "dc_m2sgan_features", "dc_m2sgan_decode",
    "dc_m2sgan_generate", "dc_m2sgan_debug_blocks", "dc_m2sgan_fold_conv",
    "dc_rhythm_create", "dc_rhythm_destroy", "dc_rhythm_psd", "dc_rhythm_contour",
    "dc_discriminator_create", "dc_discriminator_destroy", "dc_discriminator_set_param", "dc_discriminator_finalize",
    "dc_discriminator_features", "dc_discriminator_score",
]

UPDATE_CLIP_DENOISED, UPDATE_EPSILON = 1, 2
STATUS_NONFINITE, STATUS_F16_SATURATED, STATUS_TIMEOUT = 1, 2, 4
SOLVER_ROW = 12
SOLVER_ORDER = {"ddim": 1, "dpmpp2m": 2}
LOSS_TERMS = 8


class DcConfig(C.Structure):
    _fields_ = [(n, C.c_int32) for n in ("input_feats", "num_frames", "latent_dim", "ff_size", "num_layers",
                                         "num_heads", "no_eff", "precision", "max_timesteps", "device")]


class DcError(RuntimeError):
    pass


SOURCES = ("dc_kernels.hip", "dc_api.hip", "dc_music.hip", "dc_layer16.hip", "dc_stgcn.hip", "dc_m2snet.hip", "dc_loss.hip", "dc_m2sgan.hip",
           "dc_rhythm.hip")
HEADERS = ("dc_common.h", "dc_dev.h", "dc_form.h", "dc_handle.h", "dc_launch.h", "dc_mfma_f32.h", "dc_music.h", "dc_pack.h")
EXTRA_FLAGS = {}


def build_library(force: bool = False, verbose: bool = False) -> str:
    srcs = [os.path.join(CSRC, f) for f in SOURCES if os.path.exists(os.path.join(CSRC, f))]
    hdrs = [os.path.join(CSRC, f) for f in HEADERS if os.path.exists(os.path.join(CSRC, f))] + \
        [os.path.join(os.path.dirname(_HERE), "include", "dc_ddim.h")]
    hmax = max(os.path.getmtime(h) for h in hdrs)
    bdir = os.path.join(_HERE, "build")
    os.makedirs(bdir, exist_ok=True)
    hipcc = os.environ.get("HIPCC", "/opt/rocm/bin/hipcc")
    flags = ["--offload-arch=gfx950", "-O3", "-std=c++17", "-fPIC", "-fvisibility=hidden", "-Wno-unused-value"]
    objs, jobs = [], []
    for src in srcs:
        obj = os.path.join(bdir, os.path.basename(src).replace(".hip", ".o"))
        objs.append(obj)
        if force or not os.path.exists(obj) or os.path.getmtime(obj) < max(os.path.getmtime(src), hmax):
            cmd = [hipcc, *flags, *EXTRA_FLAGS.get(os.path.basename(src), []), "-c", src, "-o", obj]
            if verbose:
                print(" ".join(cmd), flush=True)
            jobs.append((cmd, subprocess.Popen(cmd)))
    for cmd, p in jobs:
        if p.wait() != 0:
            raise subprocess.CalledProcessError(p.returncode, cmd)
    if jobs or not os.path.exists(LIB_PATH) or os.path.getmtime(LIB_PATH) < max(os.path.getmtime(o) for o in objs):
        cmd = [hipcc, "--offload-arch=gfx950", "-shared", "-fPIC", *objs, "-o", LIB_PATH]
        if verbose:
            print(" ".join(cmd), flush=True)
        subprocess.run(cmd, check=True)
    return LIB_PATH


_lib = None


def lib():
    global _lib
    if _lib is not None:
        return _lib
    path = os.environ.get("DC_DDIM_LIB", LIB_PATH)
    if not os.path.exists(path):
        raise DcError(f"{path} not found: run `python -c 'import __graft_entry__ as g; g.build()'` "
                      "(there is no CPU fallback for the sampler)")
    import torch
    L = C.CDLL(path)
    L.dc_last_error.restype = C.c_char_p
    L.dc_version.restype = C.c_char_p
    L.dc_kernel_name.restype = C.c_char_p
    L.dc_kernel_name.argtypes = [C.c_int32]
    L.dc_kernel_count.restype = C.c_int32
    L.dc_sampler_workspace_bytes.restype = C.c_int64
    L.dc_sampler_workspace_bytes.argtypes = [C.c_void_p]
    L.dc_sampler_clip_stride.restype = C.c_int32
    L.dc_sampler_clip_stride.argtypes = [C.c_void_p]
    dp, fp, ip = C.POINTER(C.c_double), C.POINTER(C.c_float), C.POINTER(C.c_int32)
    L.dc_linear_beta_schedule.argtypes = [C.c_int32, dp, dp, dp, dp, dp]
    L.dc_ddim_coefficients.argtypes = [C.c_int32, dp, fp]
    L.dc_pack_weight.argtypes = [fp, C.c_int32, C.c_int32, C.c_int32, C.POINTER(C.c_uint16), C.POINTER(C.c_uint16)]
    L.dc_sampler_create.argtypes = [C.POINTER(DcConfig), C.POINTER(C.c_void_p)]
    L.dc_sampler_destroy.argtypes = [C.c_void_p]
    L.dc_sampler_destroy.restype = None
    L.dc_sampler_set_param.argtypes = [C.c_void_p, C.c_char_p, fp, C.c_int64]
    L.dc_sampler_finalize_params.argtypes = [C.c_void_p]
    L.dc_sampler_set_conditioning.argtypes = [C.c_void_p, C.c_void_p, C.c_void_p, ip, C.c_int32, C.c_int32, C.c_void_p]
    L.dc_sampler_encode_music.argtypes = [C.c_void_p, C.c_void_p, C.c_int32, C.c_int32, C.c_int32, C.c_void_p, C.c_void_p,
                                          C.c_void_p]
    L.dc_sampler_set_encoder_format.argtypes = [C.c_void_p, C.c_int32]
    L.dc_sampler_set_precise_tail.argtypes = [C.c_void_p, C.c_int32]
    L.dc_sampler_set_combine_exchange.argtypes = [C.c_void_p, C.c_int32]
    L.dc_sampler_set_clip_aligned.argtypes = [C.c_void_p, C.c_int32]
    L.dc_precise_tail_default.argtypes = [C.c_int32]
    L.dc_precise_tail_default.restype = C.c_int32
    L.dc_sampler_set_precise_forward.argtypes = [C.c_void_p, C.c_int32]
    L.dc_sampler_denoise.argtypes = [C.c_void_p, C.c_void_p, ip, C.c_void_p, C.c_void_p]
    L.dc_savgol_coefficients.argtypes = [C.c_int32, C.c_int32, fp]
    L.dc_savgol_filter.argtypes = [C.c_void_p, C.c_void_p, C.c_int32, C.c_int32, C.c_int32, C.c_int32, C.c_int32, C.c_void_p]
    L.dc_sampler_ddim_loop.argtypes = [C.c_void_p, C.c_void_p, C.c_void_p, C.c_int32, fp, ip, C.c_int32, C.c_void_p, C.c_void_p]
    L.dc_ddim_coefficients_ex.argtypes = [C.c_int32, dp, C.c_float, fp]
    L.dc_sampler_ddim_loop_ex.argtypes = [C.c_void_p, C.c_void_p, C.c_void_p, C.c_int32, fp, C.c_int32, C.c_void_p, ip, C.c_int32,
                                          C.c_void_p, C.c_void_p]
    L.dc_ddim_coefficients_known.argtypes = [C.c_int32, dp, C.c_float, fp, fp]
    L.dc_solver_table.argtypes = [C.c_int32, dp, ip, C.c_int32, C.c_float, C.c_int32, fp, fp]
    L.dc_sampler_solver_loop.argtypes = [C.c_void_p, C.c_void_p, C.c_void_p, C.c_int32, ip, fp, C.c_int32, C.c_void_p, ip, C.c_int32,
                                         C.c_void_p, C.c_void_p]
    L.dc_sampler_solver_profile_loop.argtypes = [C.c_void_p, C.c_void_p, C.c_void_p, C.c_int32, ip, fp, C.c_int32, fp, ip, C.c_int32,
                                                 C.c_void_p]
    L.dc_sampler_set_known.argtypes = [C.c_void_p, C.c_void_p, C.c_void_p, C.c_void_p]
    L.dc_sampler_set_conditioning_guided.argtypes = [C.c_void_p, C.c_void_p, C.c_void_p, ip, C.c_int32, C.c_int32, fp, fp, C.c_void_p]
    L.dc_sampler_set_guidance_scale.argtypes = [C.c_void_p, C.c_float]
    L.dc_sampler_set_conditioning_takes.argtypes = [C.c_void_p, C.c_void_p, C.c_void_p, ip, C.c_int32, C.c_int32, C.c_int32, fp, fp, C.c_void_p]
    L.dc_sampler_set_step_noise_seed.argtypes = [C.c_void_p, C.c_uint64]
    L.dc_sampler_set_step_noise_seed_at.argtypes = [C.c_void_p, C.c_uint64, C.c_uint64]
    L.dc_step_noise_fill.argtypes = [C.c_void_p, C.c_int64, C.c_uint64, C.c_int32, C.c_void_p]
    L.dc_sampler_status.argtypes = [C.c_void_p, ip, C.c_int32]
    L.dc_sampler_set_smoothing.argtypes = [C.c_void_p, C.c_int32, C.c_int32]
    L.dc_sampler_debug_denoise.argtypes = [C.c_void_p, C.c_void_p, ip, C.c_void_p, C.c_int32, C.c_int32, C.c_void_p]
    L.dc_sampler_debug_read.argtypes = [C.c_void_p, C.c_char_p, C.c_void_p, C.c_int64]
    L.dc_sampler_debug_layer.argtypes = [C.c_void_p, fp, ip, C.c_int32, C.c_int32, C.c_int32, C.c_void_p]
    L.dc_sampler_profile_loop.argtypes = [C.c_void_p, C.c_void_p, C.c_void_p, C.c_int32, fp, fp, ip, C.c_int32, C.c_void_p]
    L.dc_motion_encoder_create.argtypes = [C.c_int32, C.POINTER(C.c_void_p)]
    L.dc_motion_encoder_destroy.argtypes = [C.c_void_p]
    L.dc_motion_encoder_destroy.restype = None
    L.dc_motion_encoder_set_param.argtypes = [C.c_void_p, C.c_char_p, fp, C.c_int64]
    L.dc_motion_encoder_finalize.argtypes = [C.c_void_p]
    L.dc_motion_encoder_encode.argtypes = [C.c_void_p, C.c_void_p, C.c_int32, C.c_int32, C.c_void_p, C.c_void_p]
    L.dc_m2snet_create.argtypes = [C.c_int32, C.POINTER(C.c_void_p)]
    L.dc_m2snet_destroy.argtypes = [C.c_void_p]
    L.dc_m2snet_destroy.restype = None
    L.dc_m2snet_set_param.argtypes = [C.c_void_p, C.c_char_p, fp, C.c_int64]
    L.dc_m2snet_finalize.argtypes = [C.c_void_p]
    L.dc_m2snet_encode_music.argtypes = [C.c_void_p, C.c_void_p, C.c_int32, C.c_int32, C.c_void_p, C.c_void_p]
    L.dc_m2snet_fuse.argtypes = [C.c_void_p, C.c_void_p, C.c_void_p, C.c_int32, C.c_int32, C.c_void_p, C.c_void_p, C.c_void_p]
    L.dc_m2snet_score.argtypes = [C.c_void_p, C.c_void_p, C.c_void_p, C.c_int32, C.c_int32, C.c_int32, C.c_void_p, C.c_void_p,
                                  C.c_void_p]
    L.dc_q_sample_coefficients.argtypes = [C.c_int32, dp, ip, C.c_int32, fp, fp]
    L.dc_q_sample.argtypes = [C.c_void_p, C.c_void_p, fp, fp, C.c_int32, C.c_int32, C.c_int32, C.c_uint64, C.c_int32, C.c_uint64,
                              C.c_void_p, C.c_void_p, C.c_void_p]
    L.dc_motion_loss_terms.argtypes = [C.c_void_p, C.c_void_p, ip, C.c_int32, C.c_int32, C.c_int32, C.c_void_p, C.c_void_p]
    L.dc_latent_l1.argtypes = [C.c_void_p, C.c_void_p, C.c_int32, C.c_int32, C.c_void_p, C.c_void_p]
    L.dc_m2sgan_create.argtypes = [C.c_int32, C.POINTER(C.c_void_p)]
    L.dc_m2sgan_destroy.argtypes = [C.c_void_p]
    L.dc_m2sgan_destroy.restype = None
    L.dc_m2sgan_set_param.argtypes = [C.c_void_p, C.c_char_p, fp, C.c_int64]
    L.dc_m2sgan_finalize.argtypes = [C.c_void_p]
    L.dc_m2sgan_features.argtypes = [C.c_void_p, C.c_void_p, C.c_int32, C.c_int32, C.c_void_p, C.c_int32, C.c_void_p, C.c_void_p]
    L.dc_m2sgan_decode.argtypes = [C.c_void_p, C.c_void_p, C.c_int32, C.c_int32, C.c_void_p, C.c_void_p]
    L.dc_m2sgan_generate.argtypes = [C.c_void_p, C.c_void_p, C.c_int32, C.c_int32, C.c_void_p, C.c_int32, C.c_void_p, C.c_void_p]
    L.dc_m2sgan_debug_blocks.argtypes = [C.c_void_p, C.c_void_p, C.c_int32, C.c_int32, C.c_int32, C.c_void_p, C.c_void_p]
    L.dc_m2sgan_fold_conv.argtypes = [fp] * 7 + [C.c_int32] * 3 + [fp, fp]
    L.dc_rhythm_create.argtypes = [C.c_int32, C.POINTER(C.c_void_p)]
    L.dc_rhythm_destroy.argtypes = [C.c_void_p]
    L.dc_rhythm_destroy.restype = None
    L.dc_rhythm_psd.argtypes = [C.c_void_p, C.c_void_p, C.c_int32, C.c_int32, C.c_void_p, C.c_void_p]
    L.dc_rhythm_contour.argtypes = [C.c_void_p, C.c_void_p, C.c_int32, C.c_int32, C.c_void_p, C.c_void_p, C.c_void_p]
    L.dc_discriminator_create.argtypes = [C.c_int32, C.POINTER(C.c_void_p)]
    L.dc_discriminator_destroy.argtypes = [C.c_void_p]
    L.dc_discriminator_destroy.restype = None
    L.dc_discriminator_set_param.argtypes = [C.c_void_p, C.c_char_p, fp, C.c_int64]
    L.dc_discriminator_finalize.argtypes = [C.c_void_p]
    L.dc_discriminator_features.argtypes = [C.c_void_p, C.c_void_p, C.c_int32, C.c_int32, C.c_void_p, C.c_void_p]
    L.dc_discriminator_score.argtypes = [C.c_void_p, C.c_void_p, C.c_int32, C.c_int32, C.c_void_p, C.c_void_p]
    _lib = L
    return L


def _check(rc):
    if rc != 0:
        raise DcError(f"libdc_ddim error {rc}: {lib().dc_last_error().decode()}")


def _fptr(a):
    return a.ctypes.data_as(C.POINTER(C.c_float))

# ... 189 lines not shown
    G, NT = raw.shape[0], raw.shape[1]
    out = np.empty((G, 32, NT, 32), raw.dtype)
    lane = np.arange(64)
    for r in range(16):
        feat = tile_row(r, lane >> 5)
        out[:, lane & 31, :, feat] = raw[:, :, lane, r].transpose(2, 0, 1)
    return out.reshape(G * 32, NT * 32)


class NativeSampler:

    def __init__(self, cfg, precision="fp16", max_timesteps=1000, device=0):
        self._h = C.c_void_p()
        c = DcConfig(cfg.input_feats, cfg.num_frames, cfg.latent_dim, cfg.ff_size, cfg.num_layers, cfg.num_heads,
                     int(bool(cfg.no_eff)), DC_PREC[precision], int(max_timesteps), int(device))
        _check(lib().dc_sampler_create(C.byref(c), C.byref(self._h)))
        self.cfg, self.precision, self.device, self.max_timesteps = cfg, precision, int(device), int(max_timesteps)
        self.B = self.T = 0
        self.guided = False
        self.takes = 1

    def close(self):
        if getattr(self, "_h", None) and self._h.value:
            lib().dc_sampler_destroy(self._h)
            self._h = C.c_void_p()

    def __del__(self):
        try:
            self.close()
        except Exception:
            pass

    def load_state_dict(self, state_dict):
        for k, v in state_dict.items():
            a = v.detach().cpu().numpy() if hasattr(v, "detach") else np.asarray(v)
            if a.dtype.kind != "f":
                continue
            a = np.ascontiguousarray(a, np.float32)
            _check(lib().dc_sampler_set_param(self._h, k.encode(), _fptr(a), a.size))
        _check(lib().dc_sampler_finalize_params(self._h))

    @staticmethod
    def _stream():
        import torch
        return C.c_void_p(torch.cuda.current_stream().cuda_stream)

    def set_conditioning(self, xf_proj, xf_out, length=None, null=None, takes=1):
        import torch
        assert xf_proj.is_cuda and xf_proj.dtype == torch.float32 and xf_proj.is_contiguous()
        assert xf_out.is_cuda and xf_out.dtype == torch.float32 and xf_out.is_contiguous()
        B, T, Cc = xf_proj.shape
        assert Cc == 64 and tuple(xf_out.shape) == (B, T, 64)
        lp = None
        if length is not None:
            la = np.ascontiguousarray(np.asarray(length.cpu() if hasattr(length, "cpu") else length), np.int32)
            assert la.shape == (B,)
            lp = _iptr(la)
        nv = [None, None]
        if null is not None:
            nv = [None if v is None else
                  np.ascontiguousarray(np.asarray(v.detach().cpu() if hasattr(v, "detach") else v), np.float32).reshape(-1) for v in null]
            assert len(nv) == 2 and all(v is None or v.shape == (64,) for v in nv), "null = (null_proj[64], null_out[64])"
        if int(takes) != 1:
            _check(lib().dc_sampler_set_conditioning_takes(self._h, xf_proj.data_ptr(), xf_out.data_ptr(), lp, B, T, int(takes),
                                                           *[None if v is None else _fptr(v) for v in nv], self._stream()))
        elif null is None:
            _check(lib().dc_sampler_set_conditioning(self._h, xf_proj.data_ptr(), xf_out.data_ptr(), lp, B, T, self._stream()))
        else:
            _check(lib().dc_sampler_set_conditioning_guided(self._h, xf_proj.data_ptr(), xf_out.data_ptr(), lp, B, T,
                                                            *[None if v is None else _fptr(v) for v in nv], self._stream()))
        self.takes = int(takes)
        self.B, self.T = B * self.takes, T
        self.guided = null is not None

    def set_guidance_scale(self, w):
        _check(lib().dc_sampler_set_guidance_scale(self._h, C.c_float(float(w))))

    def set_precise_tail(self, steps):
        _check(lib().dc_sampler_set_precise_tail(self._h, int(steps)))

    def set_clip_aligned(self, mode):
        _check(lib().dc_sampler_set_clip_aligned(self._h, -1 if mode is None else (1 if mode else 0)))

    def set_precise_forward(self, on):
        _check(lib().dc_sampler_set_precise_forward(self._h, 1 if on else 0))

    def set_combine_exchange(self, on):
        _check(lib().dc_sampler_set_combine_exchange(self._h, 1 if on else 0))

    def set_encoder_format(self, fmt):
        _check(lib().dc_sampler_set_encoder_format(self._h, {"split": 0, "f16": 1, "fp16": 1}[fmt]))

    def encode_music(self, mel, out=None):
        import torch
        assert mel.is_cuda and mel.dtype == torch.float32 and mel.is_contiguous() and mel.dim() == 3
        B, Tm, nm = mel.shape
        T = (Tm - 1) // 3 + 1
        if out is None:
            xf_proj = torch.empty((B, T, 64), dtype=torch.float32, device=mel.device)
            xf_out = torch.empty_like(xf_proj)
        else:
            xf_proj, xf_out = out
            for t in out:
                assert t.is_cuda and t.dtype == torch.float32 and t.is_contiguous() and tuple(t.shape) == (B, T, 64)
        _check(lib().dc_sampler_encode_music(self._h, mel.data_ptr(), B, Tm, nm, xf_proj.data_ptr(), xf_out.data_ptr(),
                                             self._stream()))
        return xf_proj, xf_out

    def denoise(self, x, timesteps):
        import torch
        assert x.is_cuda and x.dtype == torch.float32 and x.is_contiguous()
        assert tuple(x.shape) == (self.B, self.T, self.cfg.input_feats)
        ta = np.ascontiguousarray(np.asarray(timesteps.cpu() if hasattr(timesteps, "cpu") else timesteps), np.int32)
        assert ta.shape == (self.B,)
        out = torch.empty_like(x)
        _check(lib().dc_sampler_denoise(self._h, x.data_ptr(), _iptr(ta), out.data_ptr(), self._stream()))
        return out

    def ddim_loop(self, noise, coef, snap_iters=(), flags=0, step_noise=None, noise_seed=None):
        import torch
        assert noise.is_cuda and noise.dtype == torch.float32 and noise.is_contiguous()
        assert tuple(noise.shape) == (self.B, self.T, self.cfg.input_feats)
        coef = np.ascontiguousarray(coef, np.float32)
        S = coef.shape[0]
        out = torch.empty_like(noise)
        si = np.ascontiguousarray(np.asarray(list(snap_iters), np.int32))
        snaps = torch.empty((len(si),) + tuple(noise.shape), dtype=torch.float32, device=noise.device) if len(si) else None
        sip, snp = (_iptr(si) if len(si) else None), (snaps.data_ptr() if snaps is not None else None)
        if coef.shape[1] == 4:
            assert flags == 0 and step_noise is None, "clip / epsilon / eta > 0 need the [S, 8] table of ddim_coefficients(.., eta)"
            _check(lib().dc_sampler_ddim_loop(self._h, noise.data_ptr(), out.data_ptr(), S, _fptr(coef), sip, len(si), snp, self._stream()))
        else:
            assert coef.shape[1] == 8
            zp = None
            if step_noise is not None:
                assert step_noise.is_cuda and step_noise.dtype == torch.float32 and step_noise.is_contiguous()
                assert tuple(step_noise.shape) == (S,) + tuple(noise.shape)
                zp = step_noise.data_ptr()
            elif noise_seed is not None:
                seed, first = noise_seed if isinstance(noise_seed, (tuple, list)) else (noise_seed, 0)
                _check(lib().dc_sampler_set_step_noise_seed_at(self._h, C.c_uint64(int(seed) & (2 ** 64 - 1)), C.c_uint64(int(first))))
            _check(lib().dc_sampler_ddim_loop_ex(self._h, noise.data_ptr(), out.data_ptr(), S, _fptr(coef), int(flags), zp, sip,
                                                 len(si), snp, self._stream()))
        return out, snaps

    def solver_loop(self, noise, timesteps, rows, snap_iters=(), flags=0, step_noise=None, noise_seed=None):
        import torch
        assert noise.is_cuda and noise.dtype == torch.float32 and noise.is_contiguous()
        assert tuple(noise.shape) == (self.B, self.T, self.cfg.input_feats)
        ts, rows, si, n = self._solver_args(timesteps, rows, snap_iters)
        out = torch.empty_like(noise)
        snaps = torch.empty((len(si),) + tuple(noise.shape), dtype=torch.float32, device=noise.device) if len(si) else None
        zp = None
        if step_noise is not None:
            assert step_noise.is_cuda and step_noise.dtype == torch.float32 and step_noise.is_contiguous()
            assert tuple(step_noise.shape) == (n,) + tuple(noise.shape)
            zp = step_noise.data_ptr()
        elif noise_seed is not None:
            seed, first = noise_seed if isinstance(noise_seed, (tuple, list)) else (noise_seed, 0)
            _check(lib().dc_sampler_set_step_noise_seed_at(self._h, C.c_uint64(int(seed) & (2 ** 64 - 1)), C.c_uint64(int(first))))
        _check(lib().dc_sampler_solver_loop(self._h, noise.data_ptr(), out.data_ptr(), n, _iptr(ts), _fptr(rows), int(flags), zp,
                                            _iptr(si) if len(si) else None, len(si), snaps.data_ptr() if snaps is not None else None,
                                            self._stream()))
        return out, snaps

    @staticmethod
# ... 307 lines not shown
```

### include/dc_ddim.h

```cpp
#ifndef DC_DDIM_H
#define DC_DDIM_H

#include <stdint.h>

#define DC_EXPORT __attribute__((visibility("default")))

#ifdef __cplusplus
extern "C" {
#endif

typedef struct dc_sampler dc_sampler;

typedef enum dc_status {
    DC_OK = 0,
    DC_ERR_INVALID = -1,
    DC_ERR_NO_DEVICE = -2,
    DC_ERR_HIP = -3,
    DC_ERR_PARAM = -4,
    DC_ERR_UNSUPPORTED = -5
} dc_status;

typedef enum dc_precision {
    DC_PREC_BF16 = 0,
    DC_PREC_MIXED = 1,
// ... 20 lines not shown

DC_EXPORT int dc_linear_beta_schedule(int32_t num_steps, double* h_betas, double* h_alphas_cumprod,
                            double* h_alphas_cumprod_prev, double* h_sqrt_recip_alphas_cumprod,
                            double* h_sqrt_recipm1_alphas_cumprod);

DC_EXPORT int dc_ddim_coefficients(int32_t num_steps, const double* h_alphas_cumprod, float* h_coef);

DC_EXPORT int dc_ddim_coefficients_ex(int32_t num_steps, const double* h_alphas_cumprod, float eta, float* h_coef8);

DC_EXPORT int dc_ddim_coefficients_known(int32_t num_steps, const double* h_alphas_cumprod, float eta, float* h_coef8, float* h_start2);

#define DC_SOLVER_ROW 12
DC_EXPORT int dc_solver_table(int32_t n_train, const double* h_alphas_cumprod, const int32_t* h_timesteps, int32_t n, float eta,
                              int32_t order, float* h_rows, float* h_start2);

DC_EXPORT int dc_pack_weight(const float* h_w, int32_t n_out, int32_t k_in, int32_t chained,
                   uint16_t* h_hi, uint16_t* h_lo);


DC_EXPORT int dc_sampler_create(const dc_config* cfg, dc_sampler** out);
DC_EXPORT void dc_sampler_destroy(dc_sampler* s);

DC_EXPORT int dc_sampler_set_param(dc_sampler* s, const char* name, const float* h_data, int64_t numel);

DC_EXPORT int dc_sampler_finalize_params(dc_sampler* s);

DC_EXPORT int dc_sampler_set_conditioning(dc_sampler* s, const float* d_xf_proj, const float* d_xf_out,
                                const int32_t* h_length, int32_t B, int32_t T, void* stream);

DC_EXPORT int dc_sampler_encode_music(dc_sampler* s, const float* d_mel, int32_t B, int32_t Tm, int32_t n_mels,
                            float* d_xf_proj, float* d_xf_out, void* stream);

DC_EXPORT int dc_sampler_set_precise_tail(dc_sampler* s, int32_t steps);
DC_EXPORT int32_t dc_precise_tail_default(int32_t precision);

DC_EXPORT int dc_sampler_set_precise_forward(dc_sampler* s, int32_t on);

#define DC_ME_SPLIT 0
#define DC_ME_FP16 1
DC_EXPORT int dc_sampler_set_encoder_format(dc_sampler* s, int32_t format);

DC_EXPORT int dc_sampler_denoise(dc_sampler* s, const float* d_x, const int32_t* h_timesteps,
                       float* d_out, void* stream);

DC_EXPORT int dc_sampler_ddim_loop(dc_sampler* s, const float* d_noise, float* d_out, int32_t num_steps,
                         const float* h_coef, const int32_t* h_snap_iters, int32_t n_snap,
                         float* d_snaps, void* stream);

#define DC_UPDATE_CLIP_DENOISED 1
#define DC_UPDATE_EPSILON 2
DC_EXPORT int dc_sampler_ddim_loop_ex(dc_sampler* s, const float* d_noise, float* d_out, int32_t num_steps, const float* h_coef8,
                            int32_t flags, const float* d_step_noise, const int32_t* h_snap_iters, int32_t n_snap,
                            float* d_snaps, void* stream);

DC_EXPORT int dc_sampler_solver_loop(dc_sampler* s, const float* d_noise, float* d_out, int32_t n, const int32_t* h_timesteps,
                                     const float* h_rows, int32_t flags, const float* d_step_noise, const int32_t* h_snap_iters,
                                     int32_t n_snap, float* d_snaps, void* stream);
DC_EXPORT int dc_sampler_solver_profile_loop(dc_sampler* s, const float* d_noise, float* d_out, int32_t n, const int32_t* h_timesteps,
                                             const float* h_rows, int32_t flags, float* h_ms, int32_t* h_count, int32_t n_kernels,
                                             void* stream);

DC_EXPORT int dc_sampler_set_known(dc_sampler* s, const float* d_known, const float* d_mask, const float* d_known_noise);

DC_EXPORT int dc_sampler_set_conditioning_guided(dc_sampler* s, const float* d_xf_proj, const float* d_xf_out, const int32_t* h_length,
                                       int32_t B, int32_t T, const float* h_null_proj, const float* h_null_out, void* stream);

DC_EXPORT int dc_sampler_set_conditioning_takes(dc_sampler* s, const float* d_xf_proj, const float* d_xf_out, const int32_t* h_length,
                                                int32_t B, int32_t T, int32_t takes, const float* h_null_proj, const float* h_null_out,
                                                void* stream);

DC_EXPORT int dc_sampler_set_guidance_scale(dc_sampler* s, float w);

DC_EXPORT int dc_sampler_set_step_noise_seed(dc_sampler* s, uint64_t seed);
DC_EXPORT int dc_sampler_set_step_noise_seed_at(dc_sampler* s, uint64_t seed, uint64_t first_element);
DC_EXPORT int dc_step_noise_fill(float* d_out, int64_t n, uint64_t seed, int32_t iteration, void* stream);

#define DC_STATUS_NONFINITE 1
#define DC_STATUS_F16_SATURATED 2
#define DC_STATUS_TIMEOUT 4
DC_EXPORT int dc_sampler_status(dc_sampler* s, int32_t* h_status, int32_t clear);

DC_EXPORT int dc_sampler_set_clip_aligned(dc_sampler* s, int32_t mode);

DC_EXPORT int dc_sampler_set_combine_exchange(dc_sampler* s, int32_t on);

DC_EXPORT int dc_sampler_profile_loop(dc_sampler* s, const float* d_noise, float* d_out, int32_t num_steps,
                            const float* h_coef, float* h_ms, int32_t* h_count, int32_t n, void* stream);
DC_EXPORT const char* dc_kernel_name(int32_t kernel_id);
DC_EXPORT int32_t dc_kernel_count(void);

DC_EXPORT int dc_sampler_debug_denoise(dc_sampler* s, const float* d_x, const int32_t* h_timesteps, float* d_out,
                             int32_t n_layers, int32_t stage, void* stream);
DC_EXPORT int dc_sampler_debug_read(dc_sampler* s, const char* what, void* h_out, int64_t nbytes);
DC_EXPORT int dc_sampler_debug_layer(dc_sampler* s, const float* h_h, const int32_t* h_timesteps, int32_t layer, int32_t first_stage,
                           int32_t last_stage, void* stream);

DC_EXPORT int dc_savgol_coefficients(int32_t window, int32_t order, float* h_coef);
DC_EXPORT int dc_sampler_set_smoothing(dc_sampler* s, int32_t window, int32_t order);
DC_EXPORT int dc_savgol_filter(const float* d_in, float* d_out, int32_t B, int32_t T, int32_t P, int32_t window, int32_t order,
                     void* stream);


typedef struct dc_motion_encoder dc_motion_encoder;
DC_EXPORT int dc_motion_encoder_create(int32_t device, dc_motion_encoder** out);
DC_EXPORT void dc_motion_encoder_destroy(dc_motion_encoder* e);

DC_EXPORT int dc_motion_encoder_set_param(dc_motion_encoder* e, const char* name, const float* h_data, int64_t numel);

DC_EXPORT int dc_motion_encoder_finalize(dc_motion_encoder* e);

DC_EXPORT int dc_motion_encoder_encode(dc_motion_encoder* e, const float* d_motion, int32_t B, int32_t T, float* d_out,
                                       void* stream);

typedef struct dc_m2snet dc_m2snet;
DC_EXPORT int dc_m2snet_create(int32_t device, dc_m2snet** out);
DC_EXPORT void dc_m2snet_destroy(dc_m2snet* n);

DC_EXPORT int dc_m2snet_set_param(dc_m2snet* n, const char* name, const float* h_data, int64_t numel);

DC_EXPORT int dc_m2snet_finalize(dc_m2snet* n);

DC_EXPORT int dc_m2snet_encode_music(dc_m2snet* n, const float* d_mel, int32_t B, int32_t Tm, float* d_music_latent, void* stream);

DC_EXPORT int dc_m2snet_fuse(dc_m2snet* n, const float* d_music_latent, const float* d_motion_latent, int32_t B, int32_t T,
                             float* d_prob, float* d_logit, void* stream);

DC_EXPORT int dc_m2snet_score(dc_m2snet* n, const float* d_mel, const float* d_motion, int32_t B, int32_t Tm, int32_t T,
                              float* d_prob, float* d_logit, void* stream);

typedef struct dc_m2sgan dc_m2sgan;
DC_EXPORT int dc_m2sgan_create(int32_t device, dc_m2sgan** out);
DC_EXPORT void dc_m2sgan_destroy(dc_m2sgan* g);

DC_EXPORT int dc_m2sgan_set_param(dc_m2sgan* g, const char* name, const float* h_data, int64_t numel);

DC_EXPORT int dc_m2sgan_finalize(dc_m2sgan* g);

DC_EXPORT int dc_m2sgan_features(dc_m2sgan* g, const float* d_mel, int32_t B, int32_t Tm, const float* d_noise, int32_t Ln, float* d_feat,
                                 void* stream);
DC_EXPORT int dc_m2sgan_decode(dc_m2sgan* g, const float* d_feat, int32_t B, int32_t T, float* d_pose, void* stream);
DC_EXPORT int dc_m2sgan_generate(dc_m2sgan* g, const float* d_mel, int32_t B, int32_t Tm, const float* d_noise, int32_t Ln, float* d_pose,
                                 void* stream);
DC_EXPORT int dc_m2sgan_debug_blocks(dc_m2sgan* g, const float* d_feat, int32_t B, int32_t T, int32_t n_blocks, float* d_h, void* stream);
DC_EXPORT int dc_m2sgan_fold_conv(const float* weight_g, const float* weight_v, const float* conv_bias, const float* bn_weight,
                                  const float* bn_bias, const float* bn_mean, const float* bn_var, int32_t cout, int32_t cin, int32_t k,
                                  float* h_w, float* h_b);

typedef struct dc_rhythm dc_rhythm;
DC_EXPORT int dc_rhythm_create(int32_t device, dc_rhythm** out);
DC_EXPORT void dc_rhythm_destroy(dc_rhythm* h);

DC_EXPORT int dc_rhythm_psd(dc_rhythm* h, const float* d_motion, int32_t B, int32_t T, float* d_psd, void* stream);

DC_EXPORT int dc_rhythm_contour(dc_rhythm* h, const float* d_motion, int32_t B, int32_t T, float* d_contour, float* d_sd, void* stream);

typedef struct dc_discriminator dc_discriminator;
DC_EXPORT int dc_discriminator_create(int32_t device, dc_discriminator** out);
DC_EXPORT void dc_discriminator_destroy(dc_discriminator* d);

DC_EXPORT int dc_discriminator_set_param(dc_discriminator* d, const char* name, const float* h_data, int64_t numel);

DC_EXPORT int dc_discriminator_finalize(dc_discriminator* d);

DC_EXPORT int dc_discriminator_features(dc_discriminator* d, const float* d_motion, int32_t B, int32_t T, float* d_feat, void* stream);
DC_EXPORT int dc_discriminator_score(dc_discriminator* d, const float* d_motion, int32_t B, int32_t T, float* d_out, void* stream);

// ... 21 lines not shown
```

Baseline: 1.661 million frames/s.

## Add slim idle-wave path for inactive waves in the layer kernel

Refactors the per-stage weight-image staging of k_layer into a LayerImages helper. Waves with no token work (!wm.active) now take a separate short path that only does the cooperative work: staging weights into LDS, the attention combine, the barriers, and writing the record. They skip the register-heavy compute and return early. The goal is to cut the instruction and latency overhead of inactive waves in workgroup-record launches. The path is on by default and has a setter to turn it off, and it risks barrier-count mismatches if the step sequence drifts from the main path.

```diff
diff --git a/diffusion-conductor_amd/csrc/dc_api.hip b/diffusion-conductor_amd/csrc/dc_api.hip
--- a/diffusion-conductor_amd/csrc/dc_api.hip
+++ b/diffusion-conductor_amd/csrc/dc_api.hip
@@ -139,6 +139,7 @@
     dc_music* music = nullptr;
     int me_format = -1;
     int clip_aligned = -1;
+    bool idle_wave_path = true;
     bool precise_forward = false;
     int tail_split = -1;
     bool host_only = false;
@@ -597,7 +598,7 @@
     Settings r;
     r.precision = s->cfg.precision, r.fmt = *s, r.no_eff = s->cfg.no_eff != 0, r.clip_aligned = s->clip_aligned, r.l16_own = s->l16_own;
     r.num_layers = s->cfg.num_layers, r.split_model = s->d_model_split != nullptr, r.film_w16 = s->h_model.film_w16 != nullptr;
-    r.film_w16_tail = s->h_model.film_w16_tail != nullptr, r.l16_max_units = dc_layer16_max_units();
+    r.film_w16_tail = s->h_model.film_w16_tail != nullptr, r.l16_max_units = dc_layer16_max_units(), r.idle_wave_path = s->idle_wave_path;
     return r;
 }
 int clip_stride(const dc_sampler* s, int B, int Tx) { return clip_stride(settings_of(s), Switches::read(), B, Tx, s->num_cu); }
@@ -793,7 +794,7 @@
                                                     s->d_snaps, iter_base, s->d_wslot, la.upd));
         return DC_OK;
     }
-    const DcLayerForm lf{fs, ss, f.wgr, f.narrow, f.g1_tiles, f.upc, f.rec_stride};
+    const DcLayerForm lf{fs, ss, f.wgr, f.narrow, f.g1_tiles, f.upc, f.rec_stride, f.idle_path};
     if (f.fuse_embed || f.fuse_extra || c.embedded) {
     } else if (c.dbg.first >= 0)
         LAUNCH(K_EMBED, dc_launch_front_from_h(st, fs, ss, dmod, s->d_h, s->d_recs, s->d_length, M, T, G, B, c.dbg.first));
@@ -1472,6 +1473,12 @@
     return DC_OK;
 }
 
+int dc_sampler_set_idle_wave_path(dc_sampler* s, int32_t on) {
+    if (!s) return fail(DC_ERR_INVALID, "null sampler");
+    s->idle_wave_path = on != 0;
+    return DC_OK;
+}
+
 int dc_sampler_set_precise_forward(dc_sampler* s, int32_t on) {
     if (!s) return fail(DC_ERR_INVALID, "null sampler");
     s->precise_forward = on != 0;
diff --git a/diffusion-conductor_amd/csrc/dc_form.h b/diffusion-conductor_amd/csrc/dc_form.h
--- a/diffusion-conductor_amd/csrc/dc_form.h
+++ b/diffusion-conductor_amd/csrc/dc_form.h
@@ -71,6 +71,7 @@
     bool split_model = false;
     bool film_w16 = false, film_w16_tail = false;
     int l16_max_units = 0;
+    bool idle_wave_path = true;
 };
 
 struct Hooks {
@@ -111,6 +112,7 @@
     bool shared_film = false;
     int film_groups = 0;
     int film_period = 0, film_wrap = 0;
+    bool idle_path = false;
 };
 
 struct FilmShare {
@@ -185,6 +187,7 @@
     const bool mixed_form = f.mixed_form = ss && !sf && ff == 1 && fs == 0;
     const bool wide_plain = wgr && !narrow && !ss && fuse_silu && ff == fs && quiet && !s.no_eff;
     f.embed_next = !w.no_embed_next && o.loop_mode && o.next_plain && wide_plain && !guided;
+    f.idle_path = s.idle_wave_path && wgr && !narrow && !ss && quiet && !s.no_eff;
     if (o.embedded && !(o.loop_mode && wide_plain)) {
         f.error = "internal: a step whose front work was done by its predecessor changed its launch form";
         return f;
@@ -276,7 +279,7 @@
     const FilmShare share = film_share(g.B, g.T, g.G, o.guided, o.takes, !s.fmt.split_film, w);
     const unsigned long long bits = w.bits() | (unsigned long long)(o.flags & 0xff) << 16 | (s.l16_own ? 1ull : 0ull) << 24 |
                                     (unsigned long long)((s.clip_aligned + 1) & 3) << 25 | guided_key_bits(o.guided, share.groups < g.G) |
-                                    (p.g1_loop ? 1ull : 0ull) << 39;
+                                    (s.idle_wave_path ? 0ull : 1ull) << 29 | (p.g1_loop ? 1ull : 0ull) << 39;
     const int K = steps_per_graph(o.S), replays = o.S / K;
     const auto part = [&](int split_n, int launches) {
         p.parts.push_back({K, split_n, launches, GraphKey{g.B, g.T, g.Tx, K, bits | (unsigned long long)split_n << 40, takes_key_period(share)}});
diff --git a/diffusion-conductor_amd/csrc/dc_kernels.hip b/diffusion-conductor_amd/csrc/dc_kernels.hip
--- a/diffusion-conductor_amd/csrc/dc_kernels.hip
+++ b/diffusion-conductor_amd/csrc/dc_kernels.hip
@@ -1149,6 +1149,105 @@
 #ifndef DC_SPLIT_NW
 #define DC_SPLIT_NW 8
 #endif
+#define DC_LAYER_STEPS(X) X(PROLOGUE) X(SA_APPLY) X(SA_STYL) X(CA_APPLY) X(CA_STYL) X(FFN) X(FFN_STYL) X(EMBED_NEXT) X(KEYS) X(VALUES)
+enum LayerStep : int {
+#define X(s) LS_##s,
+    DC_LAYER_STEPS(X)
+#undef X
+};
+template <class T16, bool SPLIT, bool WGR, int NW>
+struct LayerImages {
+    static constexpr int WM = SPLIT ? 2 : 1, NFW = 32 * WM, WSZ = (NFW + 1) * 1024, OFF_AF = 2 * WSZ, OFF_ER = OFF_AF + 16384;
+    using W = v8<T16>;
+    const DcModel* dm;
+    int l;
+    bool last, embed_next, wg_lds;
+    char* lds;
+    const W *a_sa, *acl;
+    int ub0, B, wave, lane;
+    DEV char* buf0() const { return lds; }
+    DEV char* buf1() const { return lds + WSZ; }
+    DEV void attn(const W* a) const {
+        if constexpr (SPLIT) {
+            stage_frags<NW>(a + (size_t)ub0 * 16 * 64, lds + OFF_AF, 16, wave, lane);
+        } else {
+            const int c1i = min(ub0 + 1, B - 1);
+            stage_frags<NW>(a + (size_t)ub0 * 16 * 64, lds + OFF_AF, 8, wave, lane);
+            stage_frags<NW>(a + (size_t)c1i * 16 * 64, lds + OFF_AF + 8192, 8, wave, lane);
+        }
+    }
+    DEV bool runs(LayerStep s) const { return s < LS_EMBED_NEXT || (s == LS_EMBED_NEXT ? embed_next : (!last || embed_next)); }
+    template <LayerStep S>
+    DEV void issue() const {
+        const DcLayer& L = dm->layer[l];
+        if constexpr (S == LS_PROLOGUE) {
+            stage_frags<NW>(L.img_sa_q, buf0(), NFW + 1, wave, lane);
+            if constexpr (!WGR)
+                if (wg_lds) attn(a_sa);
+        } else if constexpr (S == LS_SA_APPLY) {
+            stage_frags<NW>(L.img_sa_o, buf1(), NFW + 1, wave, lane);
+        } else if constexpr (S == LS_SA_STYL) {
+            stage_frags<NW>(L.img_ca_q, buf0(), NFW + 1, wave, lane);
+            if (wg_lds) attn(acl);
+        } else if constexpr (S == LS_CA_APPLY) {
+            stage_frags<NW>(L.img_ca_o, buf1(), NFW + 1, wave, lane);
+        } else if constexpr (S == LS_CA_STYL) {
+            stage_frags<NW>(L.img_ffn_w1, buf0(), 16 * WM, wave, lane);
+            stage_frags<NW>(L.img_ffn_w2, buf0() + 16 * WM * 1024, 16 * WM + 1, wave, lane);
+        } else if constexpr (S == LS_FFN) {
+            stage_frags<NW>(L.img_ffn_o, buf1(), NFW + 1, wave, lane);
+        } else if constexpr (S == LS_FFN_STYL) {
+            if (!last)
+                stage_frags<NW>(dm->layer[l + 1].img_sa_k, buf0(), NFW + 1, wave, lane);
+            else
+                stage_frags<NW>(dm->img_out, buf0(), 17, wave, lane);
+        } else if constexpr (S == LS_EMBED_NEXT) {
+            stage_frags<NW>(dm->layer[0].img_sa_k, buf1(), NFW + 1, wave, lane);
+            stage_frags<NW>(dm->img_je, lds + OFF_ER, 17, wave, lane);
+        } else if constexpr (S == LS_KEYS) {
+            if (embed_next)
+                stage_frags<NW>(dm->layer[0].img_sa_v, buf0(), NFW + 1, wave, lane);
+            else if (!last)
+                stage_frags<NW>(dm->layer[l + 1].img_sa_v, buf1(), NFW + 1, wave, lane);
+        }
+    }
+};
+template <LayerStep S>
+DEV void layer_barrier() { __syncthreads(); }
+template <LayerStep S, bool KEEP8 = false>
+DEV void layer_close() {
+    if constexpr (KEEP8)
+        stage_sync_keep8();
+    else
+        stage_sync();
+}
+
+template <class T16, int NW, class Img>
+DEV void layer_idle_wave(const Img& im, const float* __restrict__ recs_in, float* __restrict__ recs_out, const WgMap& wm, int tid, int wg) {
+    using W = v8<T16>;
+    float* mx = reinterpret_cast<float*>(im.lds + Img::OFF_AF);
+    sprio<3>();
+#define X(s)                                                                                                                   \
+    if (im.runs(LS_##s)) {                                                                                                     \
+        im.template issue<LS_##s>();                                                                                           \
+        if constexpr (LS_##s == LS_PROLOGUE)       \
+            wg_combine_attn<T16, false>(recs_in, reinterpret_cast<W*>(im.lds + Img::OFF_AF), reinterpret_cast<float*>(im.buf1()), \
+                                        im.ub0, im.B, wm.Mu, wm.Tu, tid, wg);                                                    \
+        if constexpr (LS_##s == LS_KEYS) {                      \
+            if (im.lane < 32)                                                                                                  \
+                for (int k = 0; k < 8; ++k) mx[(k * 32 + im.lane) * NW + im.wave] = -INFINITY;                                 \
+        }                                                                                                                      \
+        __builtin_amdgcn_sched_barrier(0);                                                                                     \
+        asm volatile("s_waitcnt vmcnt(0)" ::: "memory");                                                                       \
+        layer_barrier<LS_##s>();                                                                                               \
+        __builtin_amdgcn_sched_barrier(0);                                                                                     \
+    }
+    DC_LAYER_STEPS(X)
+#undef X
+    if (im.runs(LS_VALUES))
+        wg_write_record<NW>(recs_out, mx, reinterpret_cast<const f32x8*>(im.lds + Img::OFF_ER), reinterpret_cast<const f32x8*>(im.lds + Img::OFF_AF + 8192),
+                            reinterpret_cast<const float*>(im.lds + Img::OFF_ER + 8 * 8192), im.wave, im.lane, im.ub0, wm.nact, wm.Mu, wm.Tu, wg);
+}
 template <class T16, bool SPLIT, bool DBG, bool STAMP, bool WGR, bool NARROW = false, bool G1 = false >
 __global__ __launch_bounds__((NARROW || (SPLIT && DC_SPLIT_NW == 4)) ? 256 : 512, (SPLIT && DC_SPLIT_NW == 4) ? 1 : 2)
 void k_layer(const DcModel* __restrict__ dm, int l, float* __restrict__ hbuf, const f16x16* __restrict__ E, int NT,
@@ -1158,7 +1257,8 @@
              float* __restrict__ snaps, int M, int T, int G, int B, int dbg,
              unsigned long long* __restrict__ stamps, size_t rec_stride, const int* __restrict__ iter_base,
              int Tx , int upc ,
-             int e_groups , int e_period, int e_wrap, unsigned e_magic , const DcUpdate upd) {
+             int e_groups , int e_period, int e_wrap, unsigned e_magic ,
+             int idle_path , const DcUpdate upd) {
     extern __shared__ __attribute__((aligned(16))) char lds[];
     static_assert(!NARROW || (WGR && !SPLIT && !DBG), "narrow workgroups: workgroup-record form, non-split formats, no test hooks");
     constexpr int NW = NARROW ? 4 : (SPLIT ? DC_SPLIT_NW : 8);
@@ -1184,10 +1284,21 @@
 #ifndef DC_NO_EARLY_ARGS
     {
         const unsigned grid_x = gridDim.x;
-        asm("" : "+s"(T) : "s"(l), "s"(hbuf), "s"(E), "s"(recs), "s"(a_ca), "s"(NT), "s"(M), "s"(Tx), "s"(G), "s"(B), "s"(rec_stride), "s"(upc), "s"(grid_x));
+        asm("" : "+s"(T) : "s"(l), "s"(hbuf), "s"(E), "s"(recs), "s"(a_ca), "s"(NT), "s"(M), "s"(Tx), "s"(G), "s"(B), "s"(rec_stride), "s"(upc), "s"(grid_x), "s"(idle_path));
     }
 #endif
     const int nl = dm->num_layers;
+    if constexpr (WGR && !SPLIT && !NARROW && !DBG && !STAMP) {
+        const int wave_ = __builtin_amdgcn_readfirstlane((int)threadIdx.x >> 6), wg_ = wg_index();
+        const WgMap wm_ = wg_map(wg_, wave_, NW, G, M, T, B, upc);
+        if (idle_path && !wm_.active) {
+            const bool last_ = l + 1 >= nl;
+            const LayerImages<T16, SPLIT, WGR, NW> im_{dm, l, last_, last_ && out_mode == 1 && (upd.flags & DC_UPD_EMBED_NEXT) != 0, true, lds,
+                                                       a_sa, a_ca + (size_t)l * B * 16 * 64, wm_.ub0, B, wave_, (int)threadIdx.x & 63};
+            layer_idle_wave<T16, NW>(im_, recs + (size_t)(l & 1) * rec_stride, recs + (size_t)((l + 1) & 1) * rec_stride, wm_, (int)threadIdx.x, wg_);
+            return;
+        }
+    }
     f32x16 h[4];
     {
         const int g0 = wg_map(WGR ? wg_index() : (int)blockIdx.x, threadIdx.x >> 6, NW, G, M, T, B, WGR ? upc : 0).g;
@@ -1210,35 +1321,27 @@
     const bool wg_lds = WGR || (!SPLIT && T >= NW * 32);
     const int ub0 = wm.ub0;
     char* ring = lds + OFF_ER + wave * 8192;
-    auto stage_attn = [&](const W* a) {
-        if constexpr (SPLIT) {
-            stage_frags<NW>(a + (size_t)ub0 * 16 * 64, lds + OFF_AF, 16, wave, lane);
-        } else {
-            const int c1i = min(ub0 + 1, B - 1);
-            stage_frags<NW>(a + (size_t)ub0 * 16 * 64, lds + OFF_AF, 8, wave, lane);
-            stage_frags<NW>(a + (size_t)c1i * 16 * 64, lds + OFF_AF + 8192, 8, wave, lane);
-        }
-    };
     const W* af = reinterpret_cast<const W*>(lds + OFF_AF);
-    const DcLayer& L = dm->layer[l];
     const bool last = l + 1 >= nl;
     const f16x8* Eg = reinterpret_cast<const f16x8*>(E) + ((size_t)film_tile_group(g, e_period, e_wrap, e_groups, e_magic) * NT + (size_t)l * 24) * 128;
     const W* acl = a_ca + (size_t)l * B * 16 * 64;
     const float* recs_in = recs + (size_t)(l & 1) * rec_stride;
     float* recs_out = recs + (size_t)((l + 1) & 1) * rec_stride;
+    bool embed_next = false;
+    if constexpr (WGR && !SPLIT && !NARROW && !DBG) embed_next = last && out_mode == 1 && (upd.flags & DC_UPD_EMBED_NEXT) != 0;
+    const LayerImages<T16, SPLIT, WGR, NW> im{dm, l, last, embed_next, wg_lds, lds, a_sa, acl, ub0, B, wave, lane};
+    static_assert(decltype(im)::WSZ == WSZ && decltype(im)::OFF_AF == OFF_AF && decltype(im)::OFF_ER == OFF_ER, "one LDS layout");
 
     DC_STAMP(0);
     if (STAMP && stamps && blockIdx.x == 3 && (threadIdx.x & 63) == 0 && l == 3) stamps[(threadIdx.x >> 6) * 32 + 26] = __builtin_amdgcn_s_memtime();
     DC_WGSTAMP(0);
     if (STAMP && stamps && threadIdx.x == 0 && (l == 3 || l == 4) && blockIdx.x < 256) stamps[2576 + (l - 3) * 256 + blockIdx.x] = t_first;
-    stage_frags<NW>(L.img_sa_q, buf0, NFW + 1, wave, lane);
+    im.template issue<LS_PROLOGUE>();
     if constexpr (NARROW)
         wg_combine_attn_narrow<T16>(recs_in, reinterpret_cast<W*>(lds + OFF_AF), reinterpret_cast<float*>(buf1), ub0, wm.Mu, wm.Tu, tid_, wg);
     else if constexpr (WGR)
         wg_combine_attn<T16, SPLIT>(recs_in, reinterpret_cast<W*>(lds + OFF_AF), reinterpret_cast<float*>(buf1), ub0, B, wm.Mu, wm.Tu, tid_, wg,
                                     (STAMP && stamps && blockIdx.x == 3 && l == 3) ? stamps : nullptr);
-    else if (wg_lds)
-        stage_attn(a_sa);
     DC_STAMP(14);
     constexpr bool use_ring = !SPLIT;
 #ifdef DC_PROLOGUE_WAIT_ALL
@@ -1248,7 +1351,7 @@
     }
     asm volatile("s_waitcnt vmcnt(0)" ::: "memory");
     DC_STAMP(15);
-    stage_sync();
+    layer_close<LS_PROLOGUE>();
 #else
     if constexpr (use_ring) {
         ering_issue(Eg, 0, ring, lane);
@@ -1263,7 +1366,7 @@
     }
     DC_STAMP(15);
     __builtin_amdgcn_sched_barrier(0);
-    __syncthreads(); sprio<3>();
+    layer_barrier<LS_PROLOGUE>(); sprio<3>();
     __builtin_amdgcn_sched_barrier(0);
 #endif
 #ifdef DC_DIAG_HALF_SHIFT
@@ -1274,7 +1377,7 @@
 #endif
     DC_STAMP(1);
 
-    stage_frags<NW>(L.img_sa_o, buf1, NFW + 1, wave, lane);
+    im.template issue<LS_SA_APPLY>();
     EPre ep;
     constexpr bool split_pf = DC_SPLIT_STYL_PF && SPLIT && !DBG;
     EPf epf;
@@ -1294,19 +1397,17 @@
         __builtin_amdgcn_sched_barrier(0);
         epf_fetch(epf, Eg, 0, 0, lane);
         epf_fetch(epf, Eg, 1, 1, lane);
-        stage_sync_keep8();
+        layer_close<LS_SA_APPLY, true>();
     } else
-        stage_sync();
+        layer_close<LS_SA_APPLY>();
     DC_STAMP(3);
     if constexpr (use_ring) epre_landed(ep);
     if constexpr (!use_ring) {
-        stage_frags<NW>(L.img_ca_q, buf0, NFW + 1, wave, lane);
-        if (wg_lds) stage_attn(acl);
+        im.template issue<LS_SA_STYL>();
         if (!(DBG && skip_blocks >= 1)) { if constexpr (split_pf) styl_accumulate_pf<T16, SPLIT, DC_SPLIT_STYL_PF == 2>(h, y, y_rstd, y_shift, Eg, epf, c1, w1, lane, cx.hh); else styl_accumulate<T16, SPLIT, G1>(h, y, y_rstd, y_shift, Eg, c1, w1, lane, cx.hh); }
     } else {
         auto next2 = [&]() {
-            stage_frags<NW>(L.img_ca_q, buf0, NFW + 1, wave, lane);
-            if (wg_lds) stage_attn(acl);
+            im.template issue<LS_SA_STYL>();
             ering_issue(Eg + 8 * 128, 0, ring, lane);
             ering_issue(Eg + 8 * 128, 1, ring + 4096, lane);
         };
@@ -1317,9 +1418,9 @@
     }
     if constexpr (DBG) if ((dbg & 0xff) == 1) { if (active) store_h(h, hbuf, g, lane); return; }
     DC_STAMP(4);
-    stage_sync();
+    layer_close<LS_SA_STYL>();
     DC_STAMP(5);
-    stage_frags<NW>(L.img_ca_o, buf1, NFW + 1, wave, lane);
+    im.template issue<LS_CA_APPLY>();
     if constexpr (use_ring) epre_load(ep, Eg + 8 * 128, lane);
     if (DBG && skip_blocks >= 2) {
     } else if (wg_lds)
@@ -1333,18 +1434,16 @@
         __builtin_amdgcn_sched_barrier(0);
         epf_fetch(epf, Eg + 8 * 128, 0, 0, lane);
         epf_fetch(epf, Eg + 8 * 128, 1, 1, lane);
-        stage_sync_keep8();
+        layer_close<LS_CA_APPLY, true>();
     } else
-        stage_sync();
+        layer_close<LS_CA_APPLY>();
     if constexpr (use_ring) epre_landed(ep);
     if constexpr (!use_ring) {
-        stage_frags<NW>(L.img_ffn_w1, buf0, 16 * WM, wave, lane);
-        stage_frags<NW>(L.img_ffn_w2, buf0 + 16 * WM * 1024, 16 * WM + 1, wave, lane);
+        im.template issue<LS_CA_STYL>();
         if (!(DBG && skip_blocks >= 2)) { if constexpr (split_pf) styl_accumulate_pf<T16, SPLIT, DC_SPLIT_STYL_PF == 2>(h, y, y_rstd, y_shift, Eg + 8 * 128, epf, c1, w1, lane, cx.hh); else styl_accumulate<T16, SPLIT, G1>(h, y, y_rstd, y_shift, Eg + 8 * 128, c1, w1, lane, cx.hh); }
     } else {
         auto next4 = [&]() {
-            stage_frags<NW>(L.img_ffn_w1, buf0, 16 * WM, wave, lane);
-            stage_frags<NW>(L.img_ffn_w2, buf0 + 16 * WM * 1024, 16 * WM + 1, wave, lane);
+            im.template issue<LS_CA_STYL>();
             ering_issue(Eg + 16 * 128, 0, ring, lane);
             ering_issue(Eg + 16 * 128, 1, ring + 4096, lane);
         };
@@ -1355,9 +1454,9 @@
     }
     if constexpr (DBG) if ((dbg & 0xff) == 2) { if (active) store_h(h, hbuf, g, lane); return; }
     DC_STAMP(7);
-    stage_sync();
+    layer_close<LS_CA_STYL>();
     DC_STAMP(8);
-    stage_frags<NW>(L.img_ffn_o, buf1, NFW + 1, wave, lane);
+    im.template issue<LS_FFN>();
     if constexpr (use_ring) epre_load(ep, Eg + 16 * 128, lane);
     {
         f32x16 u[2];
@@ -1398,17 +1497,12 @@
         __builtin_amdgcn_sched_barrier(0);
         epf_fetch(epf, Eg + 16 * 128, 0, 0, lane);
         epf_fetch(epf, Eg + 16 * 128, 1, 1, lane);
-        stage_sync_keep8();
+        layer_close<LS_FFN, true>();
     } else
-        stage_sync();
+        layer_close<LS_FFN>();
     if constexpr (use_ring) epre_landed(ep);
     {
-        auto next_w = [&]() {
-            if (!last)
-                stage_frags<NW>(dm->layer[l + 1].img_sa_k, buf0, NFW + 1, wave, lane);
-            else
-                stage_frags<NW>(dm->img_out, buf0, 17, wave, lane);
-        };
+        auto next_w = [&]() { im.template issue<LS_FFN_STYL>(); };
         if constexpr (!use_ring) {
             next_w();
             { if constexpr (split_pf) styl_accumulate_pf<T16, SPLIT, DC_SPLIT_STYL_PF == 2>(h, y, y_rstd, y_shift, Eg + 16 * 128, epf, c1, w1, lane, cx.hh); else styl_accumulate<T16, SPLIT, G1>(h, y, y_rstd, y_shift, Eg + 16 * 128, c1, w1, lane, cx.hh); }
@@ -1418,7 +1512,7 @@
     }
     if constexpr (DBG) if ((dbg & 0xff) == 3) { if (active) store_h(h, hbuf, g, lane); return; }
     DC_STAMP(10);
-    stage_sync();
+    layer_close<LS_FFN_STYL>();
 #ifdef DC_DIAG_HALF_SHIFT
     if constexpr (WGR && !SPLIT && !NARROW && !DBG) {
         if (wave < NW / 2) { for (int i_ = 0; i_ < DC_DIAG_HALF_SHIFT; ++i_) __builtin_amdgcn_s_barrier(); }
@@ -1427,13 +1521,8 @@
 #endif
     DC_STAMP(11);
 
-    bool embed_next = false;
-    if constexpr (WGR && !SPLIT && !NARROW && !DBG) embed_next = last && out_mode == 1 && (upd.flags & DC_UPD_EMBED_NEXT) != 0;
     if (last) {
-    if (embed_next) {
-        stage_frags<NW>(dm->layer[0].img_sa_k, buf1, NFW + 1, wave, lane);
-        stage_frags<NW>(dm->img_je, lds + OFF_ER, 17, wave, lane);
-    }
+    if (embed_next) im.template issue<LS_EMBED_NEXT>();
     f32x16 x0[1];
     const int P = dm->input_feats;
     const int e_xb = min(cx.tok, M - 1) / T, e_xn = cx.tok - e_xb * T;
@@ -1459,9 +1548,9 @@
         if constexpr (WGR && !SPLIT && !NARROW && !DBG) {
             __builtin_amdgcn_sched_barrier(0);
             asm volatile("s_waitcnt vmcnt(0)" ::: "memory");
-            __syncthreads(); sprio<3>();
+            layer_barrier<LS_EMBED_NEXT>(); sprio<3>();
             __builtin_amdgcn_sched_barrier(0);
-            stage_frags<NW>(dm->layer[0].img_sa_v, buf0, NFW + 1, wave, lane);
+            im.template issue<LS_KEYS>();
             const int xb = e_xb, xn = e_xn;
             const bool live = e_live;
             {
@@ -1553,14 +1642,13 @@
     }
     }
     {
-        const DcLayer& Ln = dm->layer[last ? 0 : l + 1];
         char* const bufK = last ? buf1 : buf0;
         char* const bufV = last ? buf0 : buf1;
         const W* const wK = reinterpret_cast<const W*>(bufK);
         const W* const wV = reinterpret_cast<const W*>(bufV);
         const float* const cK = reinterpret_cast<const float*>(bufK + NFW * 1024);
         const float* const cV = reinterpret_cast<const float*>(bufV + NFW * 1024);
-        if (!last) stage_frags<NW>(Ln.img_sa_v, bufV, NFW + 1, wave, lane);
+        if (!last) im.template issue<LS_KEYS>();
         __builtin_amdgcn_sched_barrier(0);
 #ifdef DC_DIAG_NO_HSTORE
         const bool st_h = false;
@@ -1646,7 +1734,7 @@
             else
                 asm volatile("s_waitcnt vmcnt(0)" ::: "memory");
             DC_STAMP(21);
-            __syncthreads(); sprio<3>();
+            layer_barrier<LS_KEYS>(); sprio<3>();
             __builtin_amdgcn_sched_barrier(0);
             DC_STAMP(12);
 #pragma unroll
@@ -1708,7 +1796,7 @@
             }
             __builtin_amdgcn_sched_barrier(0);
             DC_STAMP(16);
-            __syncthreads(); sprio<3>();
+            layer_barrier<LS_VALUES>(); sprio<3>();
             DC_STAMP(17);
             wg_write_record<NW>(recs_out, mx, pst, xp, ss, wave, lane, ub0, wm.nact, wm.Mu, wm.Tu, wg);
         } else {
@@ -1723,7 +1811,7 @@
                 asm volatile("s_waitcnt vmcnt(16)" ::: "memory");
             else
                 asm volatile("s_waitcnt vmcnt(0)" ::: "memory");
-            __syncthreads(); sprio<3>();
+            layer_barrier<LS_KEYS>(); sprio<3>();
             __builtin_amdgcn_sched_barrier(0);
             DC_STAMP(12);
             float* rec = recs + (size_t)cx.g * 2 * DC_REC_FLOATS;
@@ -2665,14 +2753,15 @@
 
 template <class T16, bool SP, bool DBG, bool STAMP, bool WGR, bool NARROW = false, bool G1 = false>
 static hipError_t launch_layer_t(hipStream_t st, const DcLayerArgs& a, int l, const void* a_sa, const void* a_ca, int dbg,
-                                 unsigned long long* stamps, size_t rec_stride, int upc) {
+                                 unsigned long long* stamps, size_t rec_stride, int upc, bool idle_path) {
     constexpr int NW = NARROW ? 4 : (SP ? DC_SPLIT_NW : 8);
     const size_t shm = SP ? 2 * 65 * 1024 + (WGR ? 16384 + 6144 : 0) : 2 * 33 * 1024 + 16384 + 8 * 8192 + 6144;
     static unsigned long long optin_done = 0;
     if (hipError_t e = lds_optin((const void*)k_layer<T16, SP, DBG, STAMP, WGR, NARROW, G1>, (int)shm, optin_done)) return e;
     k_layer<T16, SP, DBG, STAMP, WGR, NARROW, G1><<<dim3((WGR && upc) ? a.B * upc : (a.G + NW - 1) / NW), dim3(NW * 64), shm, st>>>(
         a.dm, l, a.hbuf, (const f16x16*)a.E, a.NT, (const v8<T16>*)a_sa, (const v8<T16>*)a_ca, a.recs, a.length, a.xin, a.xout, a.out_mode,
-        a.coef_cur, a.snap_cur, a.snaps, a.M, a.T, a.G, a.B, dbg, stamps, rec_stride, a.iter_base, a.Tx, WGR ? upc : 0, a.e_groups, a.e_period, a.e_wrap, a.e_magic, a.upd);
+        a.coef_cur, a.snap_cur, a.snaps, a.M, a.T, a.G, a.B, dbg, stamps, rec_stride, a.iter_base, a.Tx, WGR ? upc : 0, a.e_groups, a.e_period, a.e_wrap, a.e_magic,
+        idle_path ? 1 : 0, a.upd);
     return hipGetLastError();
 }
 
@@ -2690,7 +2779,7 @@
 #define X(SP, DBG, STAMP, WGR, NARROW, G1)                                                                      \
     if (f.split == SP && stop == DBG && stamp == STAMP && f.wgr == WGR && f.narrow == NARROW && f.g1 == G1)     \
         return (f.fmt == 1 ? launch_layer_t<_Float16, SP, DBG, STAMP, WGR, NARROW, G1> : launch_layer_t<__bf16, SP, DBG, STAMP, WGR, NARROW, G1>)( \
-            st, a, l, a_sa, a_ca, dbg, stamps, f.rec_stride, f.upc);
+            st, a, l, a_sa, a_ca, dbg, stamps, f.rec_stride, f.upc, f.idle_path);
     LAYER_FORMS(X)
 #undef X
     return hipErrorInvalidValue;
diff --git a/diffusion-conductor_amd/csrc/dc_launch.h b/diffusion-conductor_amd/csrc/dc_launch.h
--- a/diffusion-conductor_amd/csrc/dc_launch.h
+++ b/diffusion-conductor_amd/csrc/dc_launch.h
@@ -46,6 +46,7 @@
     bool g1;
     int upc;
     size_t rec_stride;
+    bool idle_path;
 };
 hipError_t dc_launch_embed_front(hipStream_t st, const DcLayerForm& f, const DcModel* dm, const float* x, float* hbuf, float* recs,
                                  const int* length, int M, int T, int G, int B,
diff --git a/diffusion-conductor_amd/native.py b/diffusion-conductor_amd/native.py
--- a/diffusion-conductor_amd/native.py
+++ b/diffusion-conductor_amd/native.py
@@ -15,7 +15,7 @@
 EXPORTS = [
     "dc_last_error", "dc_version", "dc_linear_beta_schedule", "dc_ddim_coefficients", "dc_pack_weight",
     "dc_sampler_create", "dc_sampler_destroy", "dc_sampler_set_param", "dc_sampler_finalize_params",
-    "dc_sampler_set_conditioning", "dc_sampler_encode_music", "dc_sampler_set_encoder_format", "dc_sampler_set_precise_tail", "dc_precise_tail_default", "dc_sampler_set_precise_forward", "dc_sampler_set_combine_exchange", "dc_sampler_set_clip_aligned", "dc_sampler_denoise", "dc_sampler_ddim_loop", "dc_sampler_profile_loop",
+    "dc_sampler_set_conditioning", "dc_sampler_encode_music", "dc_sampler_set_encoder_format", "dc_sampler_set_precise_tail", "dc_precise_tail_default", "dc_sampler_set_precise_forward", "dc_sampler_set_combine_exchange", "dc_sampler_set_clip_aligned", "dc_sampler_set_idle_wave_path", "dc_sampler_denoise", "dc_sampler_ddim_loop", "dc_sampler_profile_loop",
     "dc_kernel_name", "dc_kernel_count", "dc_sampler_workspace_bytes", "dc_sampler_clip_stride", "dc_sampler_debug_denoise",
     "dc_sampler_debug_read", "dc_sampler_debug_layer", "dc_savgol_coefficients", "dc_savgol_filter",
     "dc_ddim_coefficients_ex", "dc_sampler_ddim_loop_ex", "dc_sampler_status", "dc_sampler_set_smoothing",
@@ -125,6 +125,7 @@
     L.dc_sampler_set_precise_tail.argtypes = [C.c_void_p, C.c_int32]
     L.dc_sampler_set_combine_exchange.argtypes = [C.c_void_p, C.c_int32]
     L.dc_sampler_set_clip_aligned.argtypes = [C.c_void_p, C.c_int32]
+    L.dc_sampler_set_idle_wave_path.argtypes = [C.c_void_p, C.c_int32]
     L.dc_precise_tail_default.argtypes = [C.c_int32]
     L.dc_precise_tail_default.restype = C.c_int32
     L.dc_sampler_set_precise_forward.argtypes = [C.c_void_p, C.c_int32]
@@ -480,6 +481,9 @@
     def set_clip_aligned(self, mode):
         _check(lib().dc_sampler_set_clip_aligned(self._h, -1 if mode is None else (1 if mode else 0)))
 
+    def set_idle_wave_path(self, on):
+        _check(lib().dc_sampler_set_idle_wave_path(self._h, 1 if on else 0))
+
     def set_precise_forward(self, on):
         _check(lib().dc_sampler_set_precise_forward(self._h, 1 if on else 0))
 
diff --git a/include/dc_ddim.h b/include/dc_ddim.h
--- a/include/dc_ddim.h
+++ b/include/dc_ddim.h
@@ -126,6 +126,8 @@
 
 DC_EXPORT int dc_sampler_set_clip_aligned(dc_sampler* s, int32_t mode);
 
+DC_EXPORT int dc_sampler_set_idle_wave_path(dc_sampler* s, int32_t on);
+
 DC_EXPORT int dc_sampler_set_combine_exchange(dc_sampler* s, int32_t on);
 
 DC_EXPORT int dc_sampler_profile_loop(dc_sampler* s, const float* d_noise, float* d_out, int32_t num_steps,
```

Measured after the change: 1.678 million frames/s (median of 6 runs). +1.1%, better.
